# irfanICMLL/structure_knowledge_distillation

Measured on AMD Instinct MI355X. Metric: distillation-step images/sec @512x512 (Pi+Pa+Ho), higher is better.
Workload: dtype f32; 1 GPU; BASELINE configs[2]: ResNet18-PSPNet student + frozen ResNet101-PSPNet teacher, Pi+Pa+Ho (SAGAN D, spectral norm, WGAN-GP), batch 8 per GPU, 512x512, 19 classes; global_batch=8, parallelism=dp1

## Files before the change

### include/skd_eval.h

```cpp
#ifndef SKD_EVAL_H_
#define SKD_EVAL_H_

#include "skd.h"

#ifdef __cplusplus
extern "C" {
#endif

int skd_seg_sliding(int T, int C, int h, int w, int tile_h, int tile_w, int H, int W, const float *logits,
                    const int *tiles, const int64_t *target, int ignore_index, const uint8_t *remap, uint8_t *pred,
                    double *probs, int64_t *confusion, skd_stream_t stream);

#ifdef __cplusplus
}
#endif

#endif
```

### structure_knowledge_distillation_amd/_lib.py

```python
import ctypes
import os
import re

_HERE = os.path.dirname(os.path.abspath(__file__))
LIB_PATH = os.path.join(_HERE, "libskd_hip.so")
HEADER_PATH = os.path.normpath(os.path.join(_HERE, "..", "include", "skd.h"))
EXT_HEADER_PATH = os.path.normpath(os.path.join(_HERE, "..", "include", "skd_eval.h"))

_c = ctypes
_P = _c.c_void_p
_I = _c.c_int
_L = _c.c_int64
_F = _c.c_float
_D = _c.c_double

SIGNATURES = {
    "skd_abi_version": (_I, []),
    "skd_target_arch": (_I, []),
    "skd_bn_mean_var": (_I, [_I, _I, _I, _P, _P, _P, _P]),
    "skd_bn_forward": (_I, [_I, _I, _I, _P, _P, _P, _P, _P, _P, _P, _F, _P]),
    "skd_bn_edz_eydz": (_I, [_I, _I, _I, _P, _P, _P, _P, _P, _P, _F, _P]),
    "skd_bn_backward": (_I, [_I, _I, _I, _P, _P, _P, _P, _P, _P, _P, _P, _P, _P, _F, _P]),
    "skd_leaky_relu": (_I, [_L, _P, _F, _P]),
    "skd_leaky_relu_backward": (_I, [_L, _P, _P, _F, _P]),
    "skd_elu": (_I, [_L, _P, _P]),
    "skd_elu_backward": (_I, [_L, _P, _P, _P]),
    "skd_elu_inv": (_I, [_L, _P, _P]),
    "skd_abn_workspace_floats": (_L, [_I, _I, _I]),
    "skd_abn_forward_train": (_I, [_I, _I, _I, _P, _P, _P, _P, _P, _P, _P, _F, _F, _I, _F, _P, _P]),
    "skd_abn_stats": (_I, [_I, _I, _I, _P, _P, _P, _P, _P]),
    "skd_abn_apply": (_I, [_I, _I, _I, _P, _P, _P, _P, _P, _F, _I, _F, _P]),
    "skd_abn_apply_residual": (_I, [_I, _I, _I, _P, _P, _P, _P, _P, _P, _F, _I, _F, _P]),
    "skd_abn_apply_to": (_I, [_I, _I, _I, _P, _P, _P, _P, _P, _P, _P, _F, _I, _F, _P]),
    "skd_abn_forward_train_to": (_I, [_I, _I, _I, _P, _P, _P, _P, _P, _P, _P, _P, _P, _F, _F, _I, _F, _P, _P]),
    "skd_abn_relu_backward_reduce": (_I, [_I, _I, _I, _P, _P, _P, _P, _P, _P, _P, _F, _P, _P]),
    "skd_abn_relu_backward_dx": (_I, [_I, _I, _I, _P, _P, _P, _P, _P, _P, _P, _P, _P, _P, _P, _P, _F, _P]),
    "skd_abn_apply_nhwc": (_I, [_L, _I, _P, _P, _P, _P, _P, _P, _F, _I, _F, _P]),
    "skd_abn_nhwc_workspace_floats": (_L, [_L, _I]),
    "skd_abn_stats_nhwc": (_I, [_L, _I, _P, _P, _P, _P, _P]),
    "skd_abn_apply_nhwc_to": (_I, [_L, _I, _P, _P, _P, _P, _P, _P, _P, _F, _I, _F, _P]),
    "skd_abn_forward_train_nhwc": (_I, [_L, _I, _P, _P, _P, _P, _P, _P, _P, _P, _P, _F, _F, _I, _F, _P, _P]),
    "skd_abn_backward_reduce_nhwc": (_I, [_L, _I, _P, _P, _P, _P, _P, _P, _F, _I, _F, _P, _P]),
    "skd_abn_backward_dx_nhwc": (_I, [_L, _I, _P, _P, _P, _P, _P, _P, _P, _P, _P, _P, _F, _I, _F, _I, _P]),
    "skd_abn_relu_backward_reduce_nhwc": (_I, [_L, _I, _P, _P, _P, _P, _P, _P, _P, _F, _P, _P]),
    "skd_abn_relu_backward_reduce_nhwc_x": (_I, [_L, _I, _P, _P, _P, _P, _P, _P, _P, _P, _F, _P, _P]),
    "skd_abn_relu_backward_dx_nhwc_x": (_I, [_L, _I, _P, _P, _P, _P, _P, _P, _P, _P, _P, _P, _P, _F, _I, _P]),
    "skd_abn_backward_nhwc": (_I, [_L, _I, _P, _P, _P, _P, _P, _P, _P, _P, _P, _P, _F, _I, _F, _I, _P, _P]),
    "skd_abn_relu_backward_nhwc": (_I, [_L, _I, _P, _P, _P, _P, _P, _P, _P, _P, _P, _P, _P, _P, _P, _F, _I, _P, _P]),
    "skd_abn_relu_backward_dx_nhwc": (_I, [_L, _I, _P, _P, _P, _P, _P, _P, _P, _P, _P, _P, _P, _P, _F, _I, _P]),
    "skd_abn_combine_stats": (_I, [_I, _I, _P, _P, _I, _P, _P, _P, _P, _F, _D, _P]),
    "skd_abn_update_running": (_I, [_I, _P, _P, _P, _P, _F, _D, _P]),
    "skd_abn_backward_reduce": (_I, [_I, _I, _I, _P, _P, _P, _P, _P, _P, _F, _I, _F, _P, _P]),
    "skd_abn_backward_dx": (_I, [_I, _I, _I, _P, _P, _P, _P, _P, _P, _P, _P, _P, _P, _F, _I, _F, _P]),
    "skd_abn_backward": (_I, [_I, _I, _I, _P, _P, _P, _P, _P, _P, _P, _P, _P, _P, _F, _I, _F, _I, _P, _P]),
    "skd_pixelwise_workspace_floats": (_L, [_I, _I]),
    "skd_pixelwise_loss": (_I, [_I, _I, _I, _P, _P, _P, _P, _P, _P]),
    "skd_maxpool_argmax": (_I, [_I, _I, _I, _I, _I, _P, _P, _P, _P]),
    "skd_pairwise_ldm": (_I, [_I]),
    "skd_channel_l2_normalise": (_I, [_I, _I, _I, _P, _P, _I, _P, _I, _P, _P]),
    "skd_pairwise_workspace_floats": (_L, [_I, _I]),
    "skd_pairwise_gram_loss": (_I, [_I, _I, _I, _I, _I, _P, _P, _P, _P, _P, _P]),
    "skd_pairwise_backward_workspace_floats": (_L, [_I, _I, _I]),
    "skd_pairwise_backward": (_I, [_I, _I, _I, _I, _P, _P, _P, _P, _P, _P, _P]),
    "skd_maxunpool_scatter": (_I, [_I, _I, _I, _I, _I, _P, _L, _P, _P, _P]),
    "skd_maxpool_argmax_nhwc": (_I, [_I, _I, _I, _I, _I, _I, _P, _P, _P, _P]),
    "skd_maxunpool_scatter_nhwc": (_I, [_I, _I, _I, _I, _I, _I, _P, _L, _P, _P, _P]),
    "skd_spectral_workspace_floats": (_L, [_I, _I]),
    "skd_spectral_norm_forward": (_I, [_I, _I, _P, _P, _P, _P, _P, _P, _P]),
    "skd_spectral_norm_backward": (_I, [_I, _I, _P, _P, _P, _P, _P, _P, _P, _P]),
    "skd_spectral_norm_forward_multi": (_I, [_I, _P, _P, _P, _P, _P, _P, _P, _P, _P]),
    "skd_spectral_norm_backward_multi": (_I, [_I, _P, _P, _P, _P, _P, _P, _P, _P, _P, _P]),
    "skd_ce_dsn_workspace_floats": (_L, [_I, _I, _I, _I, _I, _I]),
    "skd_ce_dsn_forward": (_I, [_I, _I, _I, _I, _I, _I, _P, _P, _P, _I, _F, _P, _P, _P, _P, _P]),
    "skd_ppm_pooled_floats": (_L, [_I, _I, _P]),
    "skd_ppm_pool": (_I, [_I, _I, _I, _I, _P, _P, _P, _P]),
    "skd_ppm_pool_backward": (_I, [_I, _I, _I, _I, _P, _P, _P, _P]),
    "skd_ppm_concat": (_I, [_I, _I, _I, _I, _I, _I, _P, _P, _P, _P, _P]),
    "skd_ppm_concat_backward": (_I, [_I, _I, _I, _I, _I, _I, _P, _P, _P, _P]),
    "skd_conv1x1_abn_supported": (_I, [_L, _I, _I]),
    "skd_conv1x1_abn_nhwc": (_I, [_L, _I, _I, _P, _P, _P, _P, _P, _P, _P, _P, _F, _I, _F, _P]),
    "skd_abn_pack_eval_params": (_I, [_I, _P, _P, _P, _P, _F, _P, _P]),
    "skd_conv1x1_abn_pro_nhwc": (_I, [_L, _I, _I, _P, _P, _P, _P, _P, _P, _P, _P, _F, _P, _I, _F, _P]),
    "skd_pairwise_small": (_I, [_I, _I, _I, _I, _P, _P, _P, _P, _P, _P]),
    "skd_cs_transform": (_I, [_I, _I, _I, _P, _P, _P, _P, _P, _P, _P, _P, _P, _I, _I, _P, _I, _P, _I, _P, _P]),
    "skd_ppm_nhwc_workspace_floats": (_L, [_I, _I, _I, _I, _I, _I, _P]),
    "skd_ppm_pool_nhwc": (_I, [_I, _I, _I, _I, _I, _P, _P, _P, _P, _P]),
    "skd_ppm_pool_backward_nhwc": (_I, [_I, _I, _I, _I, _I, _P, _P, _P, _P]),
    "skd_ppm_concat_nhwc": (_I, [_I, _I, _I, _I, _I, _I, _P, _P, _P, _P, _P]),
    "skd_ppm_concat_backward_nhwc": (_I, [_I, _I, _I, _I, _I, _I, _P, _P, _P, _P, _P, _P]),
    "skd_ppm_fold_nhwc_workspace_floats": (_L, [_I, _I, _I, _I, _I, _P]),
    "skd_ppm_fold_nhwc": (_I, [_I, _I, _I, _I, _I, _P, _P, _L, _P, _P]),
    "skd_ppm_fold_backward_nhwc": (_I, [_I, _I, _I, _I, _I, _P, _P, _P, _L, _P, _P]),
    "skd_maxpool3x3s2_nhwc": (_I, [_I, _I, _I, _I, _I, _I, _P, _P, _P, _P]),
    "skd_head1x1_supported": (_I, [_I, _I, _I]),
    "skd_head1x1_forward_nhwc": (_I, [_I, _I, _I, _I, _P, _P, _P, _P, _P]),
    "skd_head1x1_backward_workspace_floats": (_L, [_I, _I, _I, _I]),
    "skd_head1x1_backward_nhwc": (_I, [_I, _I, _I, _I, _P, _P, _P, _P, _P, _P, _P, _P]),
    "skd_maxpool3x3s2_backward_nhwc": (_I, [_I, _I, _I, _I, _I, _I, _P, _P, _P, _P]),
    "skd_abn_relu_maxpool3x3s2_nhwc": (_I, [_I, _I, _I, _I, _I, _I, _P, _P, _P, _P, _P, _F, _P, _P, _P]),
    "skd_abn_relu_maxpool3x3s2_backward_reduce_nhwc": (_I, [_I, _I, _I, _I, _I, _I, _P, _P, _P, _P, _P, _P, _P, _P, _P, _F, _P, _P]),
    "skd_abn_relu_maxpool3x3s2_backward_dx_nhwc": (_I, [_I, _I, _I, _I, _I, _I, _P, _P, _P, _P, _P, _P, _P, _P, _P, _P, _P, _P, _F,
                                                         _I, _P]),
    "skd_seg_confusion": (_I, [_I, _I, _I, _I, _I, _I, _P, _P, _I, _P, _P, _P]),
    "skd_sum_f32": (_I, [_L, _P, _P, _F, _P, _P]),
    "skd_sync_handle_bytes": (_I, []),
    "skd_sync_max_floats": (_I, []),
    "skd_sync_create": (_P, [_I, _I, _P]),
    "skd_sync_connect": (_I, [_P, _P]),
    "skd_sync_destroy": (_I, [_P]),
    "skd_sync_all_gather": (_I, [_P, _I, _P, _P, _P]),
    "skd_abn_sync_stats": (_I, [_P, _I, _P, _P, _P, _P, _P, _P, _F, _D, _P]),
    "skd_abn_sync_grad_stats": (_I, [_P, _I, _P, _P, _P]),
    "skd_sync_set_timeout": (_I, [_P, _D]),
    "skd_abn_forward_train_nhwc_sync": (_I, [_P, _L, _I, _P, _P, _P, _P, _P, _P, _P, _P, _P, _P, _F, _F, _I, _F, _D, _P, _P]),
    "skd_abn_backward_nhwc_sync": (_I, [_P, _L, _I, _P, _P, _P, _P, _P, _P, _P, _P, _P, _P, _P, _F, _I, _F, _I, _P, _P]),
    "skd_abn_relu_backward_nhwc_sync": (_I, [_P, _L, _I, _P, _P, _P, _P, _P, _P, _P, _P, _P, _P, _P, _P, _P, _P, _F, _I, _P, _P]),
    "skd_status_words": (_I, []),
    "skd_status_read": (_I, [_P]),
    "skd_status_clear": (_I, []),
    "skd_abn_set_fused_max_workgroups": (_I, [_I]),
    "skd_abn_set_fused": (_I, [_I]),
    "skd_abn_get_fused": (_I, []),
    "skd_abn_set_sync_fused": (_I, [_I]),
    "skd_abn_get_sync_fused": (_I, []),
    "skd_abn_sync_form_counts": (_I, [_P]),
}

EXT_SIGNATURES = {
    "skd_seg_sliding": (_I, [_I, _I, _I, _I, _I, _I, _I, _I, _P, _P, _P, _I, _P, _P, _P, _P, _P]),
}

_lib = None
_test_backend = None


class SkdLibraryError(RuntimeError):
    pass


def header_prototypes(path=HEADER_PATH):
    with open(path) as fh:
        text = re.sub(r"/\*.*?\*/", "", fh.read(), flags=re.S)
    return sorted(set(re.findall(r"\b(skd_[a-z0-9_]+)\s*\(", text)))


def load(path=None):
    global _lib
    if _lib is not None and path is None:
        return _lib
    path = path or LIB_PATH
    if not os.path.exists(path):
        raise SkdLibraryError(
            "libskd_hip.so not found at %s -- build it with "
            "`python -m structure_knowledge_distillation_amd.build` (there is no CPU/eager fallback)" % path)
    try:
        lib = ctypes.CDLL(path)
    except OSError as e:
        raise SkdLibraryError("cannot load %s: %s" % (path, e))
    for table in (SIGNATURES, EXT_SIGNATURES):
        for name, (res, args) in table.items():
            try:
                fn = getattr(lib, name)
            except AttributeError:
                raise SkdLibraryError("libskd_hip.so does not export %s (stale build?)" % name)
            fn.restype = res
            fn.argtypes = args
    if path == LIB_PATH:
        _lib = lib
    return lib


def get():
    if _test_backend is not None:
        return _test_backend
    if _timing is not None:
        return _TimedLib(load())
    return load()


def has_entry(name):
    return hasattr(get(), name)


_timing = None


class _TimedLib:

    def __init__(self, lib):
        self._lib = lib

    def __getattr__(self, name):
        fn = getattr(self._lib, name)
        rec = _timing.get(name) if _timing is not None else None
        if rec is None:
            return fn
        import torch

        def timed(*args):
            e0, e1 = torch.cuda.Event(enable_timing=True), torch.cuda.Event(enable_timing=True)
            e0.record()
            r = fn(*args)
            e1.record()
            rec.append((e0, e1, args[:4]))
            return r
        return timed


def enable_kernel_timing(names):
    global _timing
    _timing = {n: [] for n in names}


def disable_kernel_timing():
    global _timing
    import torch
    out = {}
    if _timing is not None:
        torch.cuda.synchronize()
        for n, recs in _timing.items():
            out[n] = [(e0.elapsed_time(e1), dims) for e0, e1, dims in recs]
    _timing = None
    return out


def install_test_backend(backend):
    global _test_backend
    _test_backend = backend


def test_backend_active():
    return _test_backend is not None


class SkdDeviceError(RuntimeError):
    """A kernel gave up waiting inside a launch (include/skd.h section 13): its outputs are NaN from there on."""


_STATUS_MEANING = {
    0: "a cross-replica InPlace-ABN exchange timed out waiting for a peer rank (SKD_SYNC_TIMEOUT_S): a rank stalled, died or "
       "called the synchronised layers in a different order; statistics are NaN from that exchange on",
    1: "the grid barrier of a one-launch InPlace-ABN pass timed out: its workgroups were not co-resident (device shared with "
       "another grid-barrier launch, partitioned or CU-masked device) -- set SKD_ABN_FUSED=0 or lower "
       "skd_abn_set_fused_max_workgroups",
}


def device_status():
    lib = get()
    n = lib.skd_status_words()
    buf = (ctypes.c_uint * n)()
    if not lib.skd_status_read(ctypes.cast(buf, ctypes.c_void_p)):
        return None
    return list(buf)


def sync_form_counts():
    buf = (ctypes.c_int64 * 2)()
    get().skd_abn_sync_form_counts(ctypes.cast(buf, ctypes.c_void_p))
    return int(buf[0]), int(buf[1])


def raise_on_device_errors():
    words = device_status()
    if words and any(words):
        get().skd_status_clear()
        what = "; ".join("%s (code 0x%08x)" % (_STATUS_MEANING.get(i, "status word %d" % i), w) for i, w in enumerate(words) if w)
        raise SkdDeviceError("structure_knowledge_distillation_amd: " + what)


def check(ok, what):
    if not ok:
        raise RuntimeError("HIP error encountered in %s" % what)


def ptr(t):
    return None if t is None else t.data_ptr()


def int_array(values):
    return (ctypes.c_int * len(values))(*[int(v) for v in values])


def ptr_array(tensors):
    return (ctypes.c_void_p * len(tensors))(*[t.data_ptr() for t in tensors])


def stream_of(t):
    if _test_backend is not None or not t.is_cuda:
        return None
    import torch
    return torch.cuda.current_stream(t.device).cuda_stream


def require_device(*tensors):
    if _test_backend is not None:
        return
    for t in tensors:
        if t is not None and not t.is_cuda:
            raise SkdLibraryError(
                "structure_knowledge_distillation_amd ops run on MI355X only: got a %s tensor "
                "(no CPU fallback exists)" % t.device)
```

### structure_knowledge_distillation_amd/csrc/conv1x1.hip

```cpp
#include <stdio.h>
#include <stdlib.h>

#include <atomic>

#include "skd_common.hpp"

namespace skd {
namespace {

typedef float f32x16 __attribute__((ext_vector_type(16)));
typedef __bf16 bf16x8 __attribute__((ext_vector_type(8)));
typedef __bf16 bf16x2 __attribute__((ext_vector_type(2)));
typedef float f32x2 __attribute__((ext_vector_type(2)));

constexpr int kTM = 128, kTN = 128, kBK = 16, kMinWG = 3;
constexpr int kQK = kBK / 4;
constexpr int kRPP = kThreads / kQK;
constexpr int kRB = kTN / kRPP;
constexpr int kPlaneChunks = 2 * 128;
constexpr int kOperandChunks = 3 * kPlaneChunks;
constexpr int kStageChunks = 2 * kOperandChunks;
constexpr size_t kConvLds = sizeof(uint4) * 2 * kStageChunks;
constexpr int kProMaxK = 512;

__device__ __forceinline__ float inv_std_of(float var, float eps) { return (var != 0.f || eps != 0.f) ? 1.f / sqrtf(var + eps) : 0.f; }

template <int TM>
struct Staging {
  float4 a[TM / kRPP], b[kRB];
};
struct ProParams {
  float4 pm, pi, pg, pb;
};

template <bool PRO, int TM>
__device__ __forceinline__ void stage_load(Staging<TM> &s, const float *__restrict__ X, const float *__restrict__ Wt, int k0,
                                           int gkq, const int64_t (&arow)[TM / kRPP], int64_t wrow0, int K) {
  const float *xa = X + k0 + gkq, *wb = Wt + k0 + gkq;
#pragma unroll
  for (int h = 0; h < TM / kRPP; ++h) s.a[h] = *reinterpret_cast<const float4 *>(xa + arow[h]);
#pragma unroll
  for (int h = 0; h < kRB; ++h) s.b[h] = *reinterpret_cast<const float4 *>(wb + wrow0 + (int64_t)(kRPP * h) * K);
}

__device__ __forceinline__ float pro_one(float x, float m, float is, float g, float b) {
  const float z = __builtin_fmaf((x - m) * is, g, b);
  return z < 0.f ? 0.f : z;
}

__device__ __forceinline__ uint32_t pack_bf16(float x, float y) {
  const f32x2 v = {x, y};
  return __builtin_bit_cast(uint32_t, __builtin_convertvector(v, bf16x2));
}
__device__ __forceinline__ float bf16_lo(uint32_t u) { return __uint_as_float(u << 16); }
__device__ __forceinline__ float bf16_hi(uint32_t u) { return __uint_as_float(u & 0xffff0000u); }

__device__ __forceinline__ void split_store(float4 v, uint2 *dst) {
  uint2 p0, p1, p2;
  p0.x = pack_bf16(v.x, v.y);
  p0.y = pack_bf16(v.z, v.w);
  v.x -= bf16_lo(p0.x); v.y -= bf16_hi(p0.x); v.z -= bf16_lo(p0.y); v.w -= bf16_hi(p0.y);
  p1.x = pack_bf16(v.x, v.y);
  p1.y = pack_bf16(v.z, v.w);
  v.x -= bf16_lo(p1.x); v.y -= bf16_hi(p1.x); v.z -= bf16_lo(p1.y); v.w -= bf16_hi(p1.y);
  p2.x = pack_bf16(v.x, v.y);
  p2.y = pack_bf16(v.z, v.w);
  dst[0] = p0;
  dst[2 * kPlaneChunks] = p1;
  dst[4 * kPlaneChunks] = p2;
}

template <bool PRO, int TM>
__device__ __forceinline__ void stage_store(const Staging<TM> s, uint4 *stage, int srow, const float *ptab, int K, int kq) {
  constexpr int kRA = TM / kRPP;
  uint2 *sa = reinterpret_cast<uint2 *>(stage) + srow, *sb = reinterpret_cast<uint2 *>(stage + kOperandChunks) + srow;
  if (PRO) {
    ProParams pp;
    pp.pm = *reinterpret_cast<const float4 *>(ptab + kq);
    pp.pi = *reinterpret_cast<const float4 *>(ptab + K + kq);
    pp.pg = *reinterpret_cast<const float4 *>(ptab + 2 * K + kq);
    pp.pb = *reinterpret_cast<const float4 *>(ptab + 3 * K + kq);
#pragma unroll
    for (int h = 0; h < kRA; ++h) {
      float4 v = s.a[h];
      v.x = pro_one(v.x, pp.pm.x, pp.pi.x, pp.pg.x, pp.pb.x);
      v.y = pro_one(v.y, pp.pm.y, pp.pi.y, pp.pg.y, pp.pb.y);
      v.z = pro_one(v.z, pp.pm.z, pp.pi.z, pp.pg.z, pp.pb.z);
      v.w = pro_one(v.w, pp.pm.w, pp.pi.w, pp.pg.w, pp.pb.w);
      split_store(v, sa + 2 * kRPP * h);
    }
  } else {
#pragma unroll
    for (int h = 0; h < kRA; ++h) split_store(s.a[h], sa + 2 * kRPP * h);
  }
#pragma unroll
  for (int h = 0; h < kRB; ++h) split_store(s.b[h], sb + 2 * kRPP * h);
}

template <int TM>
__device__ __forceinline__ void tile_mma(const uint4 *stage, f32x16 (&acc)[TM / 64][2]) {
  constexpr int WM = TM / 64;
  const int lane = threadIdx.x & (kWave - 1), wid = threadIdx.x / kWave;
  const int wi = (wid >> 1) * (TM / 2), wj = (wid & 1) * 64;
  const int half = lane >> 5, r = lane & 31;
  const uint4 *pa = stage + half * 128 + ((wi + r) ^ (half * 4));
  const uint4 *pb = stage + kOperandChunks + half * 128 + ((wj + r) ^ (half * 4));
  bf16x8 a[WM][3], b[2][3];
#pragma unroll
  for (int p = 0; p < 3; ++p) {
#pragma unroll
    for (int i = 0; i < WM; ++i) a[i][p] = __builtin_bit_cast(bf16x8, pa[p * kPlaneChunks + 32 * i]);
#pragma unroll
    for (int j = 0; j < 2; ++j) b[j][p] = __builtin_bit_cast(bf16x8, pb[p * kPlaneChunks + 32 * j]);
  }
  constexpr int kPA[6] = {0, 1, 2, 0, 1, 0}, kPB[6] = {2, 1, 0, 1, 0, 0};
#pragma unroll
  for (int t = 0; t < 6; ++t)
#pragma unroll
    for (int i = 0; i < WM; ++i)
#pragma unroll
      for (int j = 0; j < 2; ++j)
        acc[i][j] = __builtin_amdgcn_mfma_f32_32x32x16_bf16(a[i][kPA[t]], b[j][kPB[t]], acc[i][j], 0, 0, 0);
}

template <int ACT, bool HAS_RES, bool FULL, bool NT>
__device__ __forceinline__ void store_block(const f32x16 &acc, const float *__restrict__ R, float *__restrict__ Y, int64_t row0,
                                            int col, int64_t M, int N, float mu, float is, float ga, float be, float slope) {
  const int lane = threadIdx.x & (kWave - 1);
  float rv[16];
  int64_t off[16];
#pragma unroll
  for (int q = 0; q < 16; ++q) {
    const int64_t row = row0 + (q & 3) + 8 * (q >> 2) + 4 * (lane >> 5);
    off[q] = row * N + col;
    rv[q] = 0.f;
    if (HAS_RES && (FULL || row < M)) rv[q] = NT ? __builtin_nontemporal_load(R + off[q]) : R[off[q]];
  }
#pragma unroll
  for (int q = 0; q < 16; ++q) {
    const int64_t row = row0 + (q & 3) + 8 * (q >> 2) + 4 * (lane >> 5);
    float z = ((acc[q] - mu) * is) * ga + be;
    if (HAS_RES) z += rv[q];
    if (ACT == SKD_ACT_RELU) z = z < 0.f ? 0.f : z;
    if (ACT == SKD_ACT_LEAKY_RELU) z = z < 0.f ? z * slope : z;
    if (FULL || row < M) {
      if (NT) __builtin_nontemporal_store(z, Y + off[q]);
      else Y[off[q]] = z;
    }
  }
}

template <int TM, int ACT, bool HAS_RES, bool PRO, bool NT>
__device__ __forceinline__ void conv1x1_tile(const float *__restrict__ X, const float *__restrict__ Wt, const float *__restrict__ R,
                                             float *__restrict__ Y, const float *__restrict__ mean, const float *__restrict__ var,
                                             const float *__restrict__ weight, const float *__restrict__ bias,
                                             const float *__restrict__ ppack, float eps, float slope, int64_t M, int K, int N,
                                             int64_t m0, int n0, uint4 *lds) {
  constexpr int WM = TM / 64, kRA = TM / kRPP;
  f32x16 acc[WM][2];
#pragma unroll
  for (int i = 0; i < WM; ++i)
#pragma unroll
    for (int j = 0; j < 2; ++j)
#pragma unroll
      for (int q = 0; q < 16; ++q) acc[i][j][q] = 0.f;
  const int nk = K / kBK;
  const int gt = threadIdx.x, grow = gt / kQK, gkq = (gt % kQK) * 4;
  const int kh = gkq >> 3;
  const int srow = 2 * (kh * 128 + (grow ^ (kh * 4))) + ((gkq >> 2) & 1);
  int64_t arow[kRA];
#pragma unroll
  for (int h = 0; h < kRA; ++h) {
    const int64_t m = m0 + grow + kRPP * h;
    arow[h] = (m > M - 1 ? M - 1 : m) * K;
  }
  const int64_t wrow0 = (int64_t)(n0 + grow) * K;
  float *ptab = reinterpret_cast<float *>(lds + 2 * kStageChunks);
  if (PRO) {
    for (int i = gt * 4; i < 4 * K; i += kThreads * 4) *reinterpret_cast<float4 *>(ptab + i) = *reinterpret_cast<const float4 *>(ppack + i);
    __syncthreads();
  }
  Staging<TM> st;
  stage_load<PRO, TM>(st, X, Wt, 0, gkq, arow, wrow0, K);
  stage_store<PRO, TM>(st, lds, srow, ptab, K, gkq);
  __syncthreads();
  int stage = 0;
  for (int kt = 0; kt < nk; ++kt) {
    const bool more = kt + 1 < nk;
    if (more) stage_load<PRO, TM>(st, X, Wt, (kt + 1) * kBK, gkq, arow, wrow0, K);
    tile_mma<TM>(lds + stage * kStageChunks, acc);
    if (more) stage_store<PRO, TM>(st, lds + (stage ^ 1) * kStageChunks, srow, ptab, K, (kt + 1) * kBK + gkq);
    __syncthreads();
    stage ^= 1;
  }
  const int lane = threadIdx.x & (kWave - 1), wid = threadIdx.x / kWave;
  const int wi = (wid >> 1) * (TM / 2), wj = (wid & 1) * 64;
  const bool full = m0 + TM <= M;
#pragma unroll
  for (int bj = 0; bj < 2; ++bj) {
    const int col = n0 + wj + bj * 32 + (lane & 31);
    const float mu = mean[col], is = inv_std_of(var[col], eps);
    const float ga = weight != nullptr ? fabsf(weight[col]) + eps : 1.f;
    const float be = bias != nullptr ? bias[col] : 0.f;
#pragma unroll
    for (int bi = 0; bi < WM; ++bi) {
      const int64_t row0 = m0 + wi + bi * 32;
      if (full)
        store_block<ACT, HAS_RES, true, NT>(acc[bi][bj], R, Y, row0, col, M, N, mu, is, ga, be, slope);
      else
        store_block<ACT, HAS_RES, false, NT>(acc[bi][bj], R, Y, row0, col, M, N, mu, is, ga, be, slope);
    }
  }
}

template <int ACT, bool HAS_RES, bool PRO, bool NT>
__global__ __launch_bounds__(kThreads, kMinWG) void conv1x1_abn_kernel(
    const float *__restrict__ X, const float *__restrict__ Wt, const float *__restrict__ R, float *__restrict__ Y,
    const float *__restrict__ mean, const float *__restrict__ var, const float *__restrict__ weight,
    const float *__restrict__ bias, const float *__restrict__ ppack, float eps, float slope, int64_t M, int K, int N,
    int tiles_n, int pm, int ct, int p_full) {
  extern __shared__ __attribute__((aligned(16))) uint4 lds[];
  const int xcd = blockIdx.x & 7, j = blockIdx.x >> 3;
  const int per_group = pm * tiles_n;
  const int group = j / per_group, r = j - group * per_group;
  const int per_chunk = pm * ct;
  const int chunk = r / per_chunk, r2 = r - chunk * per_chunk;
  const int pl = r2 / ct;
  const int tn = chunk * ct + (r2 - pl * ct);
  const int64_t tm = ((int64_t)group * pm + pl) * 8 + xcd;
  if (tn >= tiles_n) return;
  const int n0 = tn * kTN;
  if (tm < p_full) {
    const int64_t m0 = tm * kTM;
    if (m0 >= M) return;
    conv1x1_tile<kTM, ACT, HAS_RES, PRO, NT>(X, Wt, R, Y, mean, var, weight, bias, ppack, eps, slope, M, K, N, m0, n0, lds);
  } else {
    const int64_t m0 = (int64_t)p_full * kTM + (tm - p_full) * (kTM / 2);
    if (m0 >= M) return;
    conv1x1_tile<kTM / 2, ACT, HAS_RES, PRO, NT>(X, Wt, R, Y, mean, var, weight, bias, ppack, eps, slope, M, K, N, m0, n0, lds);
  }
}

__global__ void pack_eval_params_kernel(int K, const float *__restrict__ mean, const float *__restrict__ var,
                                        const float *__restrict__ weight, const float *__restrict__ bias, float eps,
                                        float *__restrict__ pack) {
  const int k = blockIdx.x * blockDim.x + threadIdx.x;
  if (k >= K) return;
  pack[k] = mean[k];
  pack[K + k] = inv_std_of(var[k], eps);
  pack[2 * (int64_t)K + k] = weight != nullptr ? fabsf(weight[k]) + eps : 1.f;
  pack[3 * (int64_t)K + k] = bias != nullptr ? bias[k] : 0.f;
}

static int cu_count(hipStream_t st) {
  static std::atomic<int> cus[64];
  int dev = -1;
  if (hipStreamGetDevice(st, &dev) != hipSuccess) {
    (void)hipGetLastError();
    if (hipGetDevice(&dev) != hipSuccess) return 0;
  }
  if (dev < 0 || dev >= 64) return 0;
  int n = cus[dev].load(std::memory_order_relaxed);
  if (n == 0 && hipDeviceGetAttribute(&n, hipDeviceAttributeMultiprocessorCount, dev) == hipSuccess && n > 0)
    cus[dev].store(n, std::memory_order_relaxed);
  return n > 0 ? n : 0;
}

template <int ACT, bool HAS_RES, bool PRO, bool NT = false>
static int launch(const float *X, const float *Wt, const float *R, float *Y, const float *mean, const float *var,
                  const float *weight, const float *bias, const float *ppack, float eps, float slope, int64_t M, int K, int N,
                  hipStream_t st) {
  static PerDeviceFlag ready;
  bool *rdy = ready.get();
  if (rdy == nullptr) return 0;
  if (!*rdy) {
    if (hipFuncSetAttribute(reinterpret_cast<const void *>(conv1x1_abn_kernel<ACT, HAS_RES, PRO, NT>),
                            hipFuncAttributeMaxDynamicSharedMemorySize, (int)(kConvLds + sizeof(float) * 4 * kProMaxK)) != hipSuccess) return 0;
    *rdy = true;
  }
  const size_t lds_bytes = kConvLds + (PRO ? sizeof(float) * 4 * (size_t)K : 0);
  const int tiles_n = N / kTN;
  const int64_t tiles_m = cdiv(M, kTM);
  const int64_t tile_bytes = (int64_t)kTN * K * sizeof(float);
  int ct = (int)((1 << 20) / tile_bytes), pm = (int)((2 << 20) / tile_bytes);
  if (ct < 1) ct = 1;
  if (pm < 1) pm = 1;
  if (ct >= tiles_n) { ct = tiles_n; pm = 1; }
  else if (!NT) return launch<ACT, HAS_RES, PRO, true>(X, Wt, R, Y, mean, var, weight, bias, ppack, eps, slope, M, K, N, st);
  while (tiles_n % ct) --ct;
  int64_t p_full = tiles_m, panels = tiles_m;
  {
    const int64_t slots = (int64_t)kMinWG * cu_count(st);
    const int64_t tiles = tiles_m * tiles_n;
    if (slots > 0 && tiles > slots && tiles % slots != 0) {
      p_full = (tiles / slots) * slots / tiles_n / 8 * 8;
      const int64_t rest_rows = M - p_full * kTM;
      panels = p_full + cdiv(rest_rows, kTM / 2);
    }
  }
  const int64_t panels_per_xcd = cdiv(cdiv(panels, 8), pm) * pm;
  if (panels_per_xcd * 8 * tiles_n > 2147483647) return 0;
  const int64_t grid = panels_per_xcd * 8 * tiles_n;
  conv1x1_abn_kernel<ACT, HAS_RES, PRO, NT><<<dim3((unsigned)grid), dim3(kThreads), lds_bytes, st>>>(
      X, Wt, R, Y, mean, var, weight, bias, ppack, eps, slope, M, K, N, tiles_n, pm, ct, (int)p_full);
  return ok();
}

}
}

using namespace skd;

extern "C" {

int skd_conv1x1_abn_supported(int64_t M, int K, int N) { return M > 0 && K > 0 && N > 0 && K % kBK == 0 && N % kTN == 0; }

static int conv1x1_dispatch(int64_t M, int K, int N, const float *x, const float *w, const float *residual, float *out,
                            const float *mean, const float *var, const float *weight, const float *bias, const float *ppack,
                            float eps, int activation, float slope, skd_stream_t stream) {
  if (!skd_conv1x1_abn_supported(M, K, N) || !x || !w || !out || !mean || !var) return 0;
  if ((reinterpret_cast<uintptr_t>(x) | reinterpret_cast<uintptr_t>(w) | reinterpret_cast<uintptr_t>(ppack)) & 15) return 0;
  hipStream_t st = as_stream(stream);
#define SKD_C11(A)                                                                                                        \
  if (ppack != nullptr)                                                                                                   \
    return residual ? launch<A, true, true>(x, w, residual, out, mean, var, weight, bias, ppack, eps, slope, M, K, N, st)   \
                    : launch<A, false, true>(x, w, residual, out, mean, var, weight, bias, ppack, eps, slope, M, K, N, st); \
  return residual ? launch<A, true, false>(x, w, residual, out, mean, var, weight, bias, nullptr, eps, slope, M, K, N, st) \
                  : launch<A, false, false>(x, w, residual, out, mean, var, weight, bias, nullptr, eps, slope, M, K, N, st)
  switch (activation) {
    case SKD_ACT_NONE: SKD_C11(SKD_ACT_NONE);
    case SKD_ACT_RELU: SKD_C11(SKD_ACT_RELU);
    case SKD_ACT_LEAKY_RELU: SKD_C11(SKD_ACT_LEAKY_RELU);
    default: return 0;
  }
#undef SKD_C11
}

int skd_conv1x1_abn_nhwc(int64_t M, int K, int N, const float *x, const float *w, const float *residual, float *out,
                         const float *mean, const float *var, const float *weight, const float *bias, float eps,
                         int activation, float slope, skd_stream_t stream) {
  return conv1x1_dispatch(M, K, N, x, w, residual, out, mean, var, weight, bias, nullptr, eps, activation, slope, stream);
}

int skd_abn_pack_eval_params(int K, const float *mean, const float *var, const float *weight, const float *bias, float eps,
                             float *pack, skd_stream_t stream) {
  if (K <= 0 || !mean || !var || !pack) return 0;
  pack_eval_params_kernel<<<dim3((unsigned)cdiv(K, 256)), dim3(256), 0, as_stream(stream)>>>(K, mean, var, weight, bias, eps, pack);
  return ok();
}

int skd_conv1x1_abn_pro_nhwc(int64_t M, int K, int N, const float *x, const float *w, const float *residual, float *out,
                             const float *mean, const float *var, const float *weight, const float *bias, float eps,
                             const float *ppack, int activation, float slope, skd_stream_t stream) {
  if (!ppack || K > kProMaxK) return 0;
  return conv1x1_dispatch(M, K, N, x, w, residual, out, mean, var, weight, bias, ppack, eps, activation, slope, stream);
}

}
```

### structure_knowledge_distillation_amd/functional.py

```python
import ctypes

import torch
from torch.autograd import Function
from torch.autograd.function import once_differentiable

from . import _lib


def _f32c(t, what):
    if t.dtype != torch.float32:
        raise TypeError("%s: fp32 tensors only (got %s)" % (what, t.dtype))
    return t if t.is_contiguous() else t.contiguous()


class _PixelWise(Function):
    @staticmethod
    def forward(ctx, logits_s, logits_t):
        _lib.require_device(logits_s, logits_t)
        assert logits_s.shape == logits_t.shape, "the output dim of teacher and student differ"
        s, t = _f32c(logits_s, "pixel_wise_loss"), _f32c(logits_t, "pixel_wise_loss")
        n, c = s.shape[0], s.shape[1]
        hw = s.numel() // max(1, n * c)
        lib, st = _lib.get(), _lib.stream_of(s)
        loss = s.new_empty(())
        need_grad = ctx.needs_input_grad[0]
        grad = torch.empty_like(s) if need_grad else None
        ws = s.new_empty((max(1, lib.skd_pixelwise_workspace_floats(n, hw)),))
        _lib.check(lib.skd_pixelwise_loss(n, c, hw, s.data_ptr(), t.data_ptr(), loss.data_ptr(),
                                          _lib.ptr(grad), ws.data_ptr(), st), "skd_pixelwise_loss")
        ctx.save_for_backward(grad)
        return loss

    @staticmethod
    @once_differentiable
    def backward(ctx, g):
        (grad,) = ctx.saved_tensors
        return (grad * g if grad is not None else None), None


def pixel_wise_loss(logits_s, logits_t):
    return _PixelWise.apply(logits_s, logits_t.detach())


class _CrossEntropyDSN(Function):
    @staticmethod
    def forward(ctx, logits_main, logits_dsn, target, ignore_index, aux_weight):
        _lib.require_device(logits_main, logits_dsn, target)
        lm = _f32c(logits_main, "cross_entropy_dsn")
        ld = _f32c(logits_dsn, "cross_entropy_dsn") if logits_dsn is not None else None
        if target.dtype != torch.int64:
            raise TypeError("cross_entropy_dsn: int64 target expected (got %s)" % target.dtype)
        tg = target if target.is_contiguous() else target.contiguous()
        b, c, h, w = lm.shape
        if ld is not None and ld.shape != lm.shape:
            raise ValueError("main and dsn logits differ in shape")
        if tg.dim() != 3 or tg.shape[0] != b:
            raise ValueError("target must be (B, H, W)")
        H, W = tg.shape[1], tg.shape[2]
        lib, st = _lib.get(), _lib.stream_of(lm)
        need_m = ctx.needs_input_grad[0]
        need_d = ld is not None and ctx.needs_input_grad[1]
        loss = lm.new_empty(())
        gm = torch.empty_like(lm) if need_m else None
        gd = torch.empty_like(ld) if need_d else None
        ws = lm.new_empty((max(8, lib.skd_ce_dsn_workspace_floats(b, c, h, w, H, W)),))
        _lib.check(lib.skd_ce_dsn_forward(b, c, h, w, H, W, lm.data_ptr(), _lib.ptr(ld), tg.data_ptr(),
                                          int(ignore_index), float(aux_weight), loss.data_ptr(), _lib.ptr(gm),
                                          _lib.ptr(gd), ws.data_ptr(), st), "skd_ce_dsn_forward")
        ctx.save_for_backward(gm, gd)
        return loss

    @staticmethod
    @once_differentiable
    def backward(ctx, g):
        gm, gd = ctx.saved_tensors
        return (gm * g if gm is not None else None), (gd * g if gd is not None else None), None, None, None


def cross_entropy_dsn(logits_main, logits_dsn, target, ignore_index=255, aux_weight=0.4):
    return _CrossEntropyDSN.apply(logits_main, logits_dsn, target, ignore_index, aux_weight)


def _is_cl(t):
    return (t.dim() == 4 and t.shape[1] % 4 == 0 and not t.is_contiguous()
            and t.is_contiguous(memory_format=torch.channels_last))


def _cl(t):
    return t if t.is_contiguous(memory_format=torch.channels_last) else t.contiguous(memory_format=torch.channels_last)


def _new_cl(ref, b, c, h, w):
    return ref.new_empty((b, h, w, c), dtype=torch.float32).permute(0, 3, 1, 2)


class _PPMPool(Function):

    @staticmethod
    def forward(ctx, x, sizes):
        _lib.require_device(x)
        if x.dtype != torch.float32:
            raise TypeError("ppm_pool: fp32 tensors only (got %s)" % x.dtype)
        ctx.cl = _is_cl(x)
        if ctx.cl:
            b, c, h, w = x.shape
            lib, st = _lib.get(), _lib.stream_of(x)
            arr = _lib.int_array(sizes)
            total = lib.skd_ppm_pooled_floats(b * c, len(sizes), arr)
            if total <= 0:
                raise ValueError("ppm_pool: bad pyramid sizes %r" % (sizes,))
            buf = x.new_empty((total,))
            ws = x.new_empty((max(1, lib.skd_ppm_nhwc_workspace_floats(b, c, 0, h, w, len(sizes), arr)),))
            _lib.check(lib.skd_ppm_pool_nhwc(b, c, h, w, len(sizes), arr, x.data_ptr(), buf.data_ptr(), ws.data_ptr(), st),
                       "skd_ppm_pool_nhwc")
            ctx.geom = (b, c, h, w, tuple(sizes))
            outs, off = [], 0
            for s_ in sizes:
                n = b * c * s_ * s_
                outs.append(buf[off:off + n].view(b, s_, s_, c).permute(0, 3, 1, 2))
                off += n
            return tuple(outs)
        x = _f32c(x, "ppm_pool")
        b, c, h, w = x.shape
        lib, st = _lib.get(), _lib.stream_of(x)
        arr = _lib.int_array(sizes)
        total = lib.skd_ppm_pooled_floats(b * c, len(sizes), arr)
        if total <= 0:
            raise ValueError("ppm_pool: bad pyramid sizes %r" % (sizes,))
        buf = x.new_empty((total,))
        _lib.check(lib.skd_ppm_pool(b * c, h, w, len(sizes), arr, x.data_ptr(), buf.data_ptr(), st), "skd_ppm_pool")
        ctx.geom = (b, c, h, w, tuple(sizes))
        outs, off = [], 0
        for s_ in sizes:
            n = b * c * s_ * s_
            outs.append(buf[off:off + n].view(b, c, s_, s_))
            off += n
        return tuple(outs)

    @staticmethod
    @once_differentiable
    def backward(ctx, *grads):
        b, c, h, w, sizes = ctx.geom
        ref = next(g for g in grads if g is not None)
        if ctx.cl:
            flat = torch.cat([(_cl(g).permute(0, 2, 3, 1) if g is not None else ref.new_zeros((b, s_, s_, c))).reshape(-1)
                              for g, s_ in zip(grads, sizes)]).to(torch.float32)
            dx = _new_cl(ref, b, c, h, w)
            lib, st = _lib.get(), _lib.stream_of(flat)
            _lib.check(lib.skd_ppm_pool_backward_nhwc(b, c, h, w, len(sizes), _lib.int_array(sizes), flat.data_ptr(),
                                                      dx.data_ptr(), st), "skd_ppm_pool_backward_nhwc")
            return dx, None
        flat = torch.cat([(g if g is not None else ref.new_zeros((b, c, s_, s_))).reshape(-1)
                          for g, s_ in zip(grads, sizes)]).to(torch.float32)
        dx = ref.new_empty((b, c, h, w), dtype=torch.float32)
        lib, st = _lib.get(), _lib.stream_of(flat)
        _lib.check(lib.skd_ppm_pool_backward(b * c, h, w, len(sizes), _lib.int_array(sizes), flat.data_ptr(),
                                             dx.data_ptr(), st), "skd_ppm_pool_backward")
        return dx, None


def ppm_pool(x, sizes=(1, 2, 3, 6)):
    return _PPMPool.apply(x, tuple(int(s_) for s_ in sizes))


class _PPMConcat(Function):

    @staticmethod
    def forward(ctx, feats, *priors):
        _lib.require_device(feats, *priors)
        ctx.cl = _is_cl(feats) and feats.dtype == torch.float32 and all(p.dtype == torch.float32 and p.shape[1] % 4 == 0 for p in priors)
        if ctx.cl:
            b, cf, h, w = feats.shape
            cout = priors[0].shape[1]
            sizes = []
            for p in priors:
                if p.shape[0] != b or p.shape[1] != cout or p.shape[2] != p.shape[3]:
                    raise ValueError("ppm_concat: priors must be (B, Cout, s, s)")
                sizes.append(p.shape[2])
            priors = [_cl(p) for p in priors]
            lib, st = _lib.get(), _lib.stream_of(feats)
            cat = _new_cl(feats, b, len(priors) * cout + cf, h, w)
            _lib.check(lib.skd_ppm_concat_nhwc(b, cout, cf, h, w, len(sizes), _lib.int_array(sizes), _lib.ptr_array(priors),
                                               feats.data_ptr(), cat.data_ptr(), st), "skd_ppm_concat_nhwc")
            ctx.geom = (b, cout, cf, h, w, tuple(sizes))
            return cat
        feats = _f32c(feats, "ppm_concat")
        priors = [_f32c(p, "ppm_concat") for p in priors]
        b, cf, h, w = feats.shape
        cout = priors[0].shape[1]
        sizes = []
        for p in priors:
            if p.shape[0] != b or p.shape[1] != cout or p.shape[2] != p.shape[3]:
                raise ValueError("ppm_concat: priors must be (B, Cout, s, s)")
            sizes.append(p.shape[2])
        lib, st = _lib.get(), _lib.stream_of(feats)
        cat = feats.new_empty((b, len(priors) * cout + cf, h, w))
        _lib.check(lib.skd_ppm_concat(b, cout, cf, h, w, len(sizes), _lib.int_array(sizes), _lib.ptr_array(priors),
                                      feats.data_ptr(), cat.data_ptr(), st), "skd_ppm_concat")
        ctx.geom = (b, cout, cf, h, w, tuple(sizes))
        return cat

    @staticmethod
    @once_differentiable
    def backward(ctx, gcat):
        b, cout, cf, h, w, sizes = ctx.geom
        if ctx.cl:
            gcat = _cl(gcat.to(torch.float32))
            lib, st = _lib.get(), _lib.stream_of(gcat)
            arr = _lib.int_array(sizes)
            need_p = any(ctx.needs_input_grad[1:])
            gfeats = _new_cl(gcat, b, cf, h, w) if ctx.needs_input_grad[0] else None
            gpriors = [_new_cl(gcat, b, cout, s_, s_) for s_ in sizes] if need_p else None
            ws = gcat.new_empty((max(1, lib.skd_ppm_nhwc_workspace_floats(b, 0, cout, h, w, len(sizes), arr)),)) if need_p else None
            _lib.check(lib.skd_ppm_concat_backward_nhwc(b, cout, cf, h, w, len(sizes), arr, gcat.data_ptr(),
                                                        _lib.ptr_array(gpriors) if need_p else None, _lib.ptr(gfeats),
                                                        _lib.ptr(ws), st), "skd_ppm_concat_backward_nhwc")
            return (gfeats,) + (tuple(gpriors) if need_p else (None,) * len(sizes))
        gcat = _f32c(gcat, "ppm_concat backward")
        lib, st = _lib.get(), _lib.stream_of(gcat)
        gfeats = gcat[:, len(sizes) * cout:] if ctx.needs_input_grad[0] else None
        gpriors = [None] * len(sizes)
        if any(ctx.needs_input_grad[1:]):
            gpriors = [gcat.new_empty((b, cout, s_, s_)) for s_ in sizes]
            _lib.check(lib.skd_ppm_concat_backward(b, cout, cf, h, w, len(sizes), _lib.int_array(sizes),
                                                   gcat.data_ptr(), _lib.ptr_array(gpriors), st),
                       "skd_ppm_concat_backward")
        return (gfeats,) + tuple(gpriors)


def ppm_concat(priors, feats):
    return _PPMConcat.apply(feats, *priors)


def _fold_block_ptrs(z_all, b, cout, sizes):
    ptrs, row = [], 0
    ld = z_all.shape[1]
    for k, s_ in enumerate(sizes):
        ptrs.append(z_all.data_ptr() + 4 * (row * ld + k * 9 * cout))
        row += b * s_ * s_
    return (ctypes.c_void_p * len(ptrs))(*ptrs), ld


class _PPMFold(Function):

    @staticmethod
    def forward(ctx, base, sizes, z_all):
        _lib.require_device(base, z_all)
        b, cout, h, w = base.shape
        if cout % 4 or not base.is_contiguous(memory_format=torch.channels_last) or base.dtype != torch.float32:
            raise ValueError("ppm_fold: base must be a float32 channels-last (B, Cout, H, W) tensor")
        rows = b * sum(s_ * s_ for s_ in sizes)
        if z_all.dtype != torch.float32 or not z_all.is_contiguous() or tuple(z_all.shape) != (rows, len(sizes) * 9 * cout):
            raise ValueError("ppm_fold: Z must be a contiguous float32 (B * sum s^2, L * 9 * Cout) tensor")
        lib, st = _lib.get(), _lib.stream_of(base)
        ptrs, ld = _fold_block_ptrs(z_all, b, cout, sizes)
        _lib.check(lib.skd_ppm_fold_nhwc(b, cout, h, w, len(sizes), _lib.int_array(sizes), ptrs, ld, base.data_ptr(), st),
                   "skd_ppm_fold_nhwc")
        ctx.geom = (b, cout, h, w, tuple(sizes))
        ctx.zshape = z_all.shape
        ctx.mark_dirty(base)
        return base

    @staticmethod
    @once_differentiable
    def backward(ctx, gout):
        b, cout, h, w, sizes = ctx.geom
        gout = _cl(gout.to(torch.float32))
        gz = None
        if ctx.needs_input_grad[2]:
            lib, st = _lib.get(), _lib.stream_of(gout)
            arr = _lib.int_array(sizes)
            gz = gout.new_zeros(ctx.zshape)
            ptrs, ld = _fold_block_ptrs(gz, b, cout, sizes)
            ws = gout.new_empty((max(1, lib.skd_ppm_fold_nhwc_workspace_floats(b, cout, h, w, len(sizes), arr)),))
            _lib.check(lib.skd_ppm_fold_backward_nhwc(b, cout, h, w, len(sizes), arr, gout.data_ptr(), ptrs, ld,
                                                      ws.data_ptr(), st), "skd_ppm_fold_backward_nhwc")
        return gout if ctx.needs_input_grad[0] else None, None, gz


def ppm_fold_supported(feats, sizes):
    return (feats.is_cuda or _lib.test_backend_active()) and feats.dtype == torch.float32 and feats.dim() == 4 \
        and _is_cl(feats) and 3 * sum(sizes) <= 64 and len(sizes) <= 4


def ppm_fold_bottleneck(priors, feats, weight, cache=None):
    import torch.nn.functional as F
    cm = priors[0].shape[1]
    n_prior = len(priors) * cm
    cout = weight.shape[0]
    sizes = tuple(int(p.shape[2]) for p in priors)
    key = (weight.data_ptr(), weight._version, tuple(weight.shape))
    mats = cache.get("mats") if cache is not None and cache.get("key") == key else None
    if mats is None:
        wf = weight[:, n_prior:].contiguous(memory_format=torch.channels_last)
        w_all = weight[:, :n_prior].reshape(cout, len(priors), cm, 3, 3).permute(2, 1, 3, 4, 0).reshape(cm, len(priors) * 9 * cout)
        mats = (wf, w_all)
        if cache is not None and not (torch.is_grad_enabled() and weight.requires_grad):
            cache["key"], cache["mats"] = key, mats
    wf, w_all = mats
    base = F.conv2d(feats, wf, None, 1, 1)
    p_all = torch.cat([_cl(p).permute(0, 2, 3, 1).reshape(-1, cm) for p in priors], 0)
    return _PPMFold.apply(base, sizes, torch.mm(p_all, w_all))


class _MaxPool3x3s2(Function):

    @staticmethod
    def forward(ctx, x, oh, ow):
        _lib.require_device(x)
        b, c, h, w = x.shape
        lib, st = _lib.get(), _lib.stream_of(x)
        y = _new_cl(x, b, c, oh, ow)
        need = ctx.needs_input_grad[0]
        arg = torch.empty((b, oh, ow, c), dtype=torch.uint8, device=x.device) if need else None
        _lib.check(lib.skd_maxpool3x3s2_nhwc(b, c, h, w, oh, ow, x.data_ptr(), y.data_ptr(), _lib.ptr(arg), st), "skd_maxpool3x3s2_nhwc")
        ctx.geom = (b, c, h, w, oh, ow)
        if need:
            ctx.save_for_backward(arg)
        return y

    @staticmethod
    @once_differentiable
    def backward(ctx, gy):
        b, c, h, w, oh, ow = ctx.geom
        (arg,) = ctx.saved_tensors
        gy = _cl(gy.to(torch.float32))
        lib, st = _lib.get(), _lib.stream_of(gy)
        dx = _new_cl(gy, b, c, h, w)
        _lib.check(lib.skd_maxpool3x3s2_backward_nhwc(b, c, h, w, oh, ow, gy.data_ptr(), arg.data_ptr(), dx.data_ptr(), st),
                   "skd_maxpool3x3s2_backward_nhwc")
        return dx, None, None


def _pool_out(n, ceil_mode):
    o = (n + 2 - 3 + (1 if ceil_mode else 0)) // 2 + 1
    if ceil_mode and (o - 1) * 2 >= n + 1:
        o -= 1
    return o


stem_pool_out = _pool_out


def is_stem_pool(pool):
    def _pair(v):
        return tuple(v) if isinstance(v, (tuple, list)) else (v, v)
    return (isinstance(pool, torch.nn.MaxPool2d) and _pair(pool.kernel_size) == (3, 3) and _pair(pool.stride) == (2, 2)
            and _pair(pool.padding) == (1, 1) and _pair(pool.dilation) == (1, 1) and not pool.return_indices)


def max_pool_stem(x, pool):
    if (x.dtype == torch.float32 and _is_cl(x) and (x.is_cuda or _lib.test_backend_active()) and is_stem_pool(pool)):
        return _MaxPool3x3s2.apply(x, _pool_out(x.shape[2], pool.ceil_mode), _pool_out(x.shape[3], pool.ceil_mode))
    return pool(x)


class _Head1x1(Function):

    @staticmethod
    def forward(ctx, x, weight, bias):
        _lib.require_device(x, weight, bias)
        b, k, h, w = x.shape
        c = weight.shape[0]
        lib, st = _lib.get(), _lib.stream_of(x)
        wt = weight.reshape(c, k)
        wt = wt if wt.is_contiguous() else wt.contiguous()
        out = x.new_empty((b, c, h, w))
        _lib.check(lib.skd_head1x1_forward_nhwc(b, h * w, k, c, x.data_ptr(), wt.data_ptr(), _lib.ptr(bias), out.data_ptr(), st),
                   "skd_head1x1_forward_nhwc")
        ctx.save_for_backward(x, weight)
        ctx.has_bias = bias is not None
        return out

    @staticmethod
    @once_differentiable
    def backward(ctx, g):
        x, weight = ctx.saved_tensors
        b, k, h, w = x.shape
        c = weight.shape[0]
        need_x, need_w, need_b = ctx.needs_input_grad[0], ctx.needs_input_grad[1], ctx.has_bias and ctx.needs_input_grad[2]
        g = g if (g.dtype == torch.float32 and g.is_contiguous()) else g.to(torch.float32).contiguous()
        lib, st = _lib.get(), _lib.stream_of(x)
        wt = weight.reshape(c, k)
        wt = wt if wt.is_contiguous() else wt.contiguous()
        gx = _new_cl(x, b, k, h, w) if need_x else None
        gw = torch.empty_like(wt) if need_w else None
        gb = x.new_empty((c,)) if need_b else None
        ws = x.new_empty((max(1, lib.skd_head1x1_backward_workspace_floats(b, h * w, k, c)),))
        _lib.check(lib.skd_head1x1_backward_nhwc(b, h * w, k, c, x.data_ptr(), wt.data_ptr(), g.data_ptr(), _lib.ptr(gx), _lib.ptr(gw),
                                                 _lib.ptr(gb), ws.data_ptr(), st), "skd_head1x1_backward_nhwc")
        return gx, (gw.view_as(weight) if gw is not None else None), gb


def head1x1_supported(x, conv):
    if not (x.dtype == torch.float32 and x.dim() == 4 and _is_cl(x) and (x.is_cuda or _lib.test_backend_active())):
        return False
    if not (conv.kernel_size == (1, 1) and conv.stride == (1, 1) and conv.padding == (0, 0) and conv.dilation == (1, 1)
            and conv.groups == 1 and conv.padding_mode == "zeros" and conv.weight.dtype == torch.float32):
        return False
    grad = torch.is_grad_enabled() and (x.requires_grad or conv.weight.requires_grad
                                        or (conv.bias is not None and conv.bias.requires_grad))
    return bool(_lib.get().skd_head1x1_supported(conv.in_channels, conv.out_channels, 1 if grad else 0))


def head1x1(x, conv):
    return _Head1x1.apply(x, conv.weight, conv.bias)


def blas_1x1_bn_supported(x, conv):
    return (not torch.is_grad_enabled() and x.dtype == torch.float32 and x.dim() == 4
            and x.is_contiguous(memory_format=torch.channels_last) and conv.kernel_size == (1, 1) and conv.stride == (1, 1)
            and conv.padding == (0, 0) and conv.groups == 1 and conv.bias is None
            and conv.in_channels >= 128 and conv.out_channels >= 128)


def conv1x1_bn_blas(x, conv, bn, relu):
    key = tuple((t.data_ptr(), t._version) for t in (conv.weight, bn.weight, bn.bias, bn.running_mean, bn.running_var) if t is not None)
    fold = getattr(bn, "_blas_fold", None)
    if fold is None or fold[0] != key:
        gamma = (bn.weight.abs() + bn.eps) if bn.weight is not None else torch.ones_like(bn.running_var)
        scale = gamma / torch.sqrt(bn.running_var + bn.eps)
        w2 = (conv.weight.reshape(conv.out_channels, conv.in_channels) * scale.view(-1, 1)).contiguous()
        b2 = (bn.bias if bn.bias is not None else torch.zeros_like(scale)) - bn.running_mean * scale
        fold = (key, w2, b2.contiguous())
        bn._blas_fold = fold
    _, w2, b2 = fold
    b, _, h, w = x.shape
    x2 = x.permute(0, 2, 3, 1).reshape(b * h * w, conv.in_channels)
    out = torch._addmm_activation(b2, x2, w2.t()) if relu else torch.addmm(b2, x2, w2.t())
    return out.view(b, h, w, conv.out_channels).permute(0, 3, 1, 2)


def conv1x1_abn_supported(x, conv):
    if not ((x.is_cuda or _lib.test_backend_active()) and x.dtype == torch.float32 and x.dim() == 4
            and x.is_contiguous(memory_format=torch.channels_last)):
        return False
    if not (conv.kernel_size == (1, 1) and conv.stride == (1, 1) and conv.padding == (0, 0) and conv.groups == 1
            and conv.bias is None and conv.weight.dtype == torch.float32):
        return False
    m = x.shape[0] * x.shape[2] * x.shape[3]
    return bool(_lib.get().skd_conv1x1_abn_supported(m, conv.in_channels, conv.out_channels))


def abn_pack_eval_params(bn):
    key = tuple((t.data_ptr(), t._version) if t is not None else None
                for t in (bn.running_mean, bn.running_var, bn.weight, bn.bias)) + (float(bn.eps),)
    cached = getattr(bn, "_skd_eval_pack", None)
    if cached is not None and cached[0] == key:
        return cached[1]
    c = bn.running_mean.numel()
    pack = bn.running_mean.new_empty((4, c))
    _lib.check(_lib.get().skd_abn_pack_eval_params(c, bn.running_mean.data_ptr(), bn.running_var.data_ptr(), _lib.ptr(bn.weight),
                                                   _lib.ptr(bn.bias), float(bn.eps), pack.data_ptr(), _lib.stream_of(pack)),
               "skd_abn_pack_eval_params")
    bn._skd_eval_pack = (key, pack)
    return pack


def conv1x1_abn_eval(x, conv_weight, running_mean, running_var, weight, bias, eps=1e-5, activation="relu", slope=0.01,
                     residual=None, pro=None):
    if torch.is_grad_enabled() and (x.requires_grad or conv_weight.requires_grad):
        raise RuntimeError("conv1x1_abn_eval is inference-only")
    _lib.require_device(x, conv_weight, running_mean, running_var, weight, bias, residual)
    act = {"none": 0, "leaky_relu": 1, "relu": 3}[activation]
    b, k, h, w = x.shape
    n = conv_weight.shape[0]
    out = _new_cl(x, b, n, h, w)
    if residual is not None:
        residual = _cl(residual)
        if tuple(residual.shape) != (b, n, h, w):
            raise ValueError("residual shape %s != output shape %s" % (tuple(residual.shape), (b, n, h, w)))
    wt = conv_weight.reshape(n, k)
    if not wt.is_contiguous():
        wt = wt.contiguous()
    if pro is not None:
        _lib.require_device(pro)
        if pro.dtype != torch.float32 or tuple(pro.shape) != (4, k) or not pro.is_contiguous():
            raise ValueError("pro must be the (4, Cin) fp32 pack of abn_pack_eval_params")
        _lib.check(_lib.get().skd_conv1x1_abn_pro_nhwc(b * h * w, k, n, x.data_ptr(), wt.data_ptr(), _lib.ptr(residual), out.data_ptr(),
                                                       running_mean.data_ptr(), running_var.data_ptr(), _lib.ptr(weight),
                                                       _lib.ptr(bias), float(eps), pro.data_ptr(), act, float(slope),
                                                       _lib.stream_of(x)), "skd_conv1x1_abn_pro_nhwc")
        return out
    _lib.check(_lib.get().skd_conv1x1_abn_nhwc(b * h * w, k, n, x.data_ptr(), wt.data_ptr(), _lib.ptr(residual), out.data_ptr(),
                                               running_mean.data_ptr(), running_var.data_ptr(), _lib.ptr(weight), _lib.ptr(bias),
                                               float(eps), act, float(slope), _lib.stream_of(x)), "skd_conv1x1_abn_nhwc")
    return out


def seg_confusion(logits, target=None, ignore_index=255, confusion=None, want_pred=True):
    _lib.require_device(logits, target, confusion)
    lg = _f32c(logits.detach(), "seg_confusion")
    b, c, h, w = lg.shape
    if target is not None:
        if target.dtype != torch.int64:
            raise TypeError("seg_confusion: int64 target expected (got %s)" % target.dtype)
        tg = target if target.is_contiguous() else target.contiguous()
        H, W = tg.shape[1], tg.shape[2]
        if confusion is None:
            confusion = torch.zeros((c, c), dtype=torch.int64, device=lg.device)
    else:
        tg = None
        H, W = want_pred
    pred = torch.empty((b, H, W), dtype=torch.uint8, device=lg.device) if want_pred else None
    _lib.check(_lib.get().skd_seg_confusion(b, c, h, w, H, W, lg.data_ptr(), _lib.ptr(tg), int(ignore_index), _lib.ptr(pred),
                                            _lib.ptr(confusion), _lib.stream_of(lg)), "skd_seg_confusion")
    return pred, confusion


SEG_SLIDING_MAX_CLASSES = 32


def seg_sliding(logits, tiles, tile_size, out_size, target=None, ignore_index=255, confusion=None, remap=None, want_pred=True,
                want_probs=False):
    _lib.require_device(logits, target, confusion, remap)
    if not _lib.has_entry("skd_seg_sliding"):
        raise NotImplementedError("the active back-end does not provide skd_seg_sliding (include/skd_eval.h)")
    lg = _f32c(logits.detach(), "seg_sliding")
    if lg.dim() != 4:
        raise ValueError("seg_sliding: logits (T, C, h, w) expected (got %s)" % (tuple(lg.shape),))
    nt, c, h, w = lg.shape
    if not 1 <= c <= SEG_SLIDING_MAX_CLASSES:
        raise ValueError("seg_sliding: 1 <= classes <= %d (got %d)" % (SEG_SLIDING_MAX_CLASSES, c))
    (th, tw), (H, W) = (int(v) for v in tile_size), (int(v) for v in out_size)
    if min(th, tw, H, W) <= 0:
        raise ValueError("seg_sliding: tile_size and out_size must be positive")
    if torch.is_tensor(tiles):
        if tiles.dtype != torch.int32 or tiles.device != lg.device or tuple(tiles.shape) != (nt, 4):
            raise TypeError("seg_sliding: tiles tensor must be (%d, 4) int32 on %s" % (nt, lg.device))
        tl = tiles if tiles.is_contiguous() else tiles.contiguous()
    else:
        rows = [tuple(int(v) for v in t) for t in tiles]
        if len(rows) != nt:
            raise ValueError("seg_sliding: %d tiles for %d logit maps" % (len(rows), nt))
        for y1, x1, y2, x2 in rows:
            if not (0 <= y1 < y2 <= H and 0 <= x1 < x2 <= W and y2 - y1 <= th and x2 - x1 <= tw):
                raise ValueError("seg_sliding: tile (%d, %d, %d, %d) does not fit a %d x %d image with %d x %d tiles"
                                 % (y1, x1, y2, x2, H, W, th, tw))
        tl = torch.tensor(rows, dtype=torch.int32).reshape(nt, 4).to(lg.device)
    if target is not None:
        if target.dtype != torch.int64:
            raise TypeError("seg_sliding: int64 target expected (got %s)" % target.dtype)
        if tuple(target.shape[-2:]) != (H, W) or target.numel() != H * W:
            raise ValueError("seg_sliding: target %s does not match out_size %s" % (tuple(target.shape), (H, W)))
        tg = target if target.is_contiguous() else target.contiguous()
        if confusion is None:
            confusion = torch.zeros((c, c), dtype=torch.int64, device=lg.device)
    else:
        tg = None
    if confusion is not None and (confusion.dtype != torch.int64 or tuple(confusion.shape) != (c, c) or not confusion.is_contiguous()):
        raise TypeError("seg_sliding: confusion must be a contiguous (%d, %d) int64 tensor" % (c, c))
    if remap is not None and (remap.dtype != torch.uint8 or remap.numel() != 256 or not remap.is_contiguous()):
        raise TypeError("seg_sliding: remap must be 256 contiguous uint8 entries")
    pred = torch.empty((H, W), dtype=torch.uint8, device=lg.device) if want_pred else None
    probs = torch.empty((H, W, c), dtype=torch.float64, device=lg.device) if want_probs else None
    _lib.check(_lib.get().skd_seg_sliding(nt, c, h, w, th, tw, H, W, lg.data_ptr(), tl.data_ptr(), _lib.ptr(tg), int(ignore_index),
                                          _lib.ptr(remap), _lib.ptr(pred), _lib.ptr(probs), _lib.ptr(confusion), _lib.stream_of(lg)),
               "skd_seg_sliding")
    return pred, probs, confusion


def pool_out_size(n, k):
    return -(-n // k)


class _MaxPoolArgmax(Function):
    @staticmethod
    def forward(ctx, x, kh, kw):
        _lib.require_device(x)
        x = _f32c(x, "max_pool_argmax")
        b, c, h, w = x.shape
        oh, ow = pool_out_size(h, kh), pool_out_size(w, kw)
        lib, st = _lib.get(), _lib.stream_of(x)
        pooled = x.new_empty((b, c, oh, ow))
        need = ctx.needs_input_grad[0]
        index = torch.empty((b, c, oh, ow), dtype=torch.int32, device=x.device) if need else None
        _lib.check(lib.skd_maxpool_argmax(b * c, h, w, kh, kw, x.data_ptr(), pooled.data_ptr(),
                                          _lib.ptr(index), st), "skd_maxpool_argmax")
        ctx.geom = (b, c, h, w, kh, kw)
        ctx.save_for_backward(index)
        return pooled

    @staticmethod
    @once_differentiable
    def backward(ctx, g):
        (index,) = ctx.saved_tensors
        if index is None:
            return None, None, None
        b, c, h, w, kh, kw = ctx.geom
        g = _f32c(g, "max_pool_argmax backward")
        m = g.shape[2] * g.shape[3]
        dx = g.new_empty((b, c, h, w))
        lib, st = _lib.get(), _lib.stream_of(g)
        _lib.check(lib.skd_maxunpool_scatter(b * c, h, w, kh, kw, g.data_ptr(), m, index.data_ptr(),
                                             dx.data_ptr(), st), "skd_maxunpool_scatter")
        return dx, None, None


def max_pool_argmax(x, kh, kw, return_indices=False):
    return _MaxPoolArgmax.apply(x, int(kh), int(kw))


def max_pool_indices(x, kh, kw):
    _lib.require_device(x)
    x = _f32c(x, "max_pool_indices")
    b, c, h, w = x.shape
    oh, ow = pool_out_size(h, kh), pool_out_size(w, kw)
    pooled = x.new_empty((b, c, oh, ow))
    index = torch.empty((b, c, oh, ow), dtype=torch.int32, device=x.device)
    _lib.check(_lib.get().skd_maxpool_argmax(b * c, h, w, int(kh), int(kw), x.data_ptr(), pooled.data_ptr(),
                                             index.data_ptr(), _lib.stream_of(x)), "skd_maxpool_argmax")
    return pooled, index


class _SimDis(Function):

    @staticmethod
    def forward(ctx, f_s, f_t):
        _lib.require_device(f_s, f_t)
        f_s, f_t = _f32c(f_s, "sim_dis"), _f32c(f_t, "sim_dis")
        b, cs = f_s.shape[0], f_s.shape[1]
        ct = f_t.shape[1]
        m = f_t.shape[-1] * f_t.shape[-2]
        assert f_s.shape[0] == f_t.shape[0] and f_s.shape[2:] == f_t.shape[2:]
        lib, st = _lib.get(), _lib.stream_of(f_s)
        ldm = lib.skd_pairwise_ldm(m)
        need = ctx.needs_input_grad[0]
        fh_s = f_s.new_empty((b, cs, ldm))
        fh_t = f_s.new_empty((b, ct, ldm))
        norm_s = f_s.new_empty((b, m)) if need else None
        _lib.check(lib.skd_channel_l2_normalise(b, cs, m, f_s.data_ptr(), fh_s.data_ptr(), ldm,
                                                None, 0, _lib.ptr(norm_s), st),
                   "skd_channel_l2_normalise")
        _lib.check(lib.skd_channel_l2_normalise(b, ct, m, f_t.data_ptr(), fh_t.data_ptr(), ldm,
                                                None, 0, None, st), "skd_channel_l2_normalise")
        g = f_s.new_empty((b, ldm, ldm)) if need else None
        loss = f_s.new_empty(())
        ws = f_s.new_empty((max(1, lib.skd_pairwise_workspace_floats(b, m)),))
        _lib.check(lib.skd_pairwise_gram_loss(b, cs, ct, m, ldm, fh_s.data_ptr(), fh_t.data_ptr(),
                                              _lib.ptr(g), loss.data_ptr(), ws.data_ptr(), st),
                   "skd_pairwise_gram_loss")
        ctx.geom = (tuple(f_s.shape), m, ldm)
        ctx.save_for_backward(fh_s if need else None, g, norm_s)
        return loss

    @staticmethod
    @once_differentiable
    def backward(ctx, gl):
        fh_s, g, norm_s = ctx.saved_tensors
        if g is None:
            return None, None
        shape, m, ldm = ctx.geom
        b, cs = shape[0], shape[1]
        lib, st = _lib.get(), _lib.stream_of(g)
        gl = gl.to(torch.float32).contiguous()
        dp = g.new_empty((b, cs, ldm))
        ws = g.new_empty((max(1, lib.skd_pairwise_backward_workspace_floats(b, cs, m)),))
        _lib.check(lib.skd_pairwise_backward(b, cs, m, ldm, fh_s.data_ptr(), g.data_ptr(),
                                             norm_s.data_ptr(), gl.data_ptr(), dp.data_ptr(), ws.data_ptr(), st),
                   "skd_pairwise_backward")
        return dp[:, :, :m].reshape(shape), None


def sim_dis(f_s, f_t):
    return _SimDis.apply(f_s, f_t.detach())


def _channels_last_quads(t):
    return (t.dim() == 4 and t.shape[1] % 4 == 0 and t.is_contiguous(memory_format=torch.channels_last) and not t.is_contiguous()
            and t.data_ptr() % 16 == 0)


def _pool_feature(lib, t, kh, kw, pooled, index, st):
    b, c, h, w = t.shape
    if _channels_last_quads(t):
        _lib.check(lib.skd_maxpool_argmax_nhwc(b, c, h, w, kh, kw, t.data_ptr(), pooled.data_ptr(), _lib.ptr(index), st),
                   "skd_maxpool_argmax_nhwc")
        return t
    t = t if t.is_contiguous() else t.contiguous()
    _lib.check(lib.skd_maxpool_argmax(b * c, h, w, kh, kw, t.data_ptr(), pooled.data_ptr(), _lib.ptr(index), st), "skd_maxpool_argmax")
    return t


def _unpool_feature(lib, nhwc, geom, dp, ldp, index, st):
    b, cs, h, w, kh, kw = geom
    if nhwc:
        dx = torch.empty_strided((b, cs, h, w), (h * w * cs, 1, w * cs, cs), dtype=dp.dtype, device=dp.device)
        _lib.check(lib.skd_maxunpool_scatter_nhwc(b, cs, h, w, kh, kw, dp.data_ptr(), ldp, index.data_ptr(), dx.data_ptr(), st),
                   "skd_maxunpool_scatter_nhwc")
        return dx
    dx = dp.new_empty((b, cs, h, w))
    _lib.check(lib.skd_maxunpool_scatter(b * cs, h, w, kh, kw, dp.data_ptr(), ldp, index.data_ptr(), dx.data_ptr(), st),
               "skd_maxunpool_scatter")
    return dx


class _PairWise(Function):

    @staticmethod
    def forward(ctx, feat_s, feat_t, kh, kw):
        _lib.require_device(feat_s, feat_t)
        for t in (feat_s, feat_t):
            if t.dtype != torch.float32:
                raise TypeError("pair_wise_loss: fp32 tensors only (got %s)" % t.dtype)
        b, cs, h, w = feat_s.shape
        ct = feat_t.shape[1]
        assert feat_t.shape[0] == b and tuple(feat_t.shape[2:]) == (h, w)
        oh, ow = pool_out_size(h, kh), pool_out_size(w, kw)
        m = oh * ow
        lib, st = _lib.get(), _lib.stream_of(feat_s)
        need = ctx.needs_input_grad[0]
        ctx.nhwc = _channels_last_quads(feat_s)
        if m <= 64:
            p_s, p_t = feat_s.new_empty((b, cs, m)), feat_s.new_empty((b, ct, m))
            index = torch.empty((b, cs, m), dtype=torch.int32, device=feat_s.device) if need else None
            _pool_feature(lib, feat_s, kh, kw, p_s, index, st)
            _pool_feature(lib, feat_t, kh, kw, p_t, None, st)
            loss = feat_s.new_empty(())
            dp = feat_s.new_empty((b, cs, m)) if need else None
            ws = feat_s.new_empty((b,))
            _lib.check(lib.skd_pairwise_small(b, cs, ct, m, p_s.data_ptr(), p_t.data_ptr(), loss.data_ptr(), _lib.ptr(dp),
                                              ws.data_ptr(), st), "skd_pairwise_small")
            ctx.geom = (b, cs, h, w, kh, kw, m, 0, 0)
            ctx.small = True
            ctx.save_for_backward(dp, index)
            return loss
        ctx.small = False
        ldm = lib.skd_pairwise_ldm(m)
        p_s = feat_s.new_empty((b, cs, m))
        p_t = feat_s.new_empty((b, ct, m))
        index = torch.empty((b, cs, m), dtype=torch.int32, device=feat_s.device) if need else None
        _pool_feature(lib, feat_s, kh, kw, p_s, index, st)
        _pool_feature(lib, feat_t, kh, kw, p_t, None, st)
        fh_s = feat_s.new_empty((b, cs, ldm))
        fh_t = feat_s.new_empty((b, ct, ldm))
        norm_s = feat_s.new_empty((b, m)) if need else None
        _lib.check(lib.skd_channel_l2_normalise(b, cs, m, p_s.data_ptr(), fh_s.data_ptr(), ldm,
                                                None, 0, _lib.ptr(norm_s), st),
                   "skd_channel_l2_normalise")
        _lib.check(lib.skd_channel_l2_normalise(b, ct, m, p_t.data_ptr(), fh_t.data_ptr(), ldm,
                                                None, 0, None, st), "skd_channel_l2_normalise")
        g = feat_s.new_empty((b, ldm, ldm)) if need else None
        loss = feat_s.new_empty(())
        ws = feat_s.new_empty((max(1, lib.skd_pairwise_workspace_floats(b, m)),))
        _lib.check(lib.skd_pairwise_gram_loss(b, cs, ct, m, ldm, fh_s.data_ptr(), fh_t.data_ptr(),
                                              _lib.ptr(g), loss.data_ptr(), ws.data_ptr(), st),
                   "skd_pairwise_gram_loss")
        ctx.geom = (b, cs, h, w, kh, kw, m, ldm, 0)
        ctx.save_for_backward(fh_s if need else None, g, norm_s, index)
        return loss

    @staticmethod
    @once_differentiable
    def backward(ctx, gl):
        if ctx.small:
            dp, index = ctx.saved_tensors
            if dp is None:
                return None, None, None, None
            b, cs, h, w, kh, kw, m, _, _ = ctx.geom
            lib, st = _lib.get(), _lib.stream_of(dp)
            dpg = dp * gl.to(torch.float32)
            return _unpool_feature(lib, ctx.nhwc, (b, cs, h, w, kh, kw), dpg, m, index, st), None, None, None
        fh_s, g, norm_s, index = ctx.saved_tensors
        if g is None:
            return None, None, None, None
        b, cs, h, w, kh, kw, m, ldm, _ = ctx.geom
        lib, st = _lib.get(), _lib.stream_of(g)
        gl = gl.to(torch.float32).contiguous()
        dp = g.new_empty((b, cs, ldm))
        ws = g.new_empty((max(1, lib.skd_pairwise_backward_workspace_floats(b, cs, m)),))
        _lib.check(lib.skd_pairwise_backward(b, cs, m, ldm, fh_s.data_ptr(), g.data_ptr(),
                                             norm_s.data_ptr(), gl.data_ptr(), dp.data_ptr(), ws.data_ptr(), st),
                   "skd_pairwise_backward")
        return _unpool_feature(lib, ctx.nhwc, (b, cs, h, w, kh, kw), dp, ldm, index, st), None, None, None


def pair_wise_loss(feat_s, feat_t, kh, kw):
    return _PairWise.apply(feat_s, feat_t.detach(), int(kh), int(kw))


class _SpectralNormalize(Function):

    @staticmethod
    def forward(ctx, w_bar, u, v):
        _lib.require_device(w_bar, u, v)
        wb = _f32c(w_bar, "spectral_normalize")
        h = wb.shape[0]
        wd = wb.numel() // h
        if not (u.is_contiguous() and v.is_contiguous()) or u.numel() != h or v.numel() != wd:
            raise ValueError("spectral_normalize: u/v must be contiguous vectors of length (out, in*kh*kw)")
        lib, st = _lib.get(), _lib.stream_of(wb)
        sigma = wb.new_empty(())
        w = torch.empty_like(wb)
        ws = wb.new_empty((max(1, lib.skd_spectral_workspace_floats(h, wd)),))
        _lib.check(lib.skd_spectral_norm_forward(h, wd, wb.data_ptr(), u.data_ptr(), v.data_ptr(),
                                                 sigma.data_ptr(), w.data_ptr(), ws.data_ptr(), st),
                   "skd_spectral_norm_forward")
        ctx.u, ctx.v = u, v
        ctx.save_for_backward(wb, sigma)
        return w

    @staticmethod
    @once_differentiable
    def backward(ctx, gw):
        wb, sigma = ctx.saved_tensors
        h = wb.shape[0]
        wd = wb.numel() // h
        gw = _f32c(gw, "spectral_normalize backward")
        lib, st = _lib.get(), _lib.stream_of(wb)
        gwb = torch.empty_like(wb)
        ws = wb.new_empty((max(1, lib.skd_spectral_workspace_floats(h, wd)),))
        _lib.check(lib.skd_spectral_norm_backward(h, wd, wb.data_ptr(), ctx.u.data_ptr(), ctx.v.data_ptr(),
                                                  sigma.data_ptr(), gw.data_ptr(), gwb.data_ptr(),
                                                  ws.data_ptr(), st), "skd_spectral_norm_backward")
        return gwb, None, None


def spectral_normalize(w_bar, u, v):
    return _SpectralNormalize.apply(w_bar, u, v)


class _SpectralNormalizeMulti(Function):

    @staticmethod
    def forward(ctx, us, vs, *w_bars):
        _lib.require_device(*w_bars, *us, *vs)
        wbs = [_f32c(w, "spectral_normalize_multi") for w in w_bars]
        hs = [w.shape[0] for w in wbs]
        ws_ = [w.numel() // h for w, h in zip(wbs, hs)]
        for u, v, h, wd in zip(us, vs, hs, ws_):
            if not (u.is_contiguous() and v.is_contiguous()) or u.numel() != h or v.numel() != wd:
                raise ValueError("spectral_normalize: u/v must be contiguous vectors of length (out, in*kh*kw)")
        lib, st = _lib.get(), _lib.stream_of(wbs[0])
        sigmas = wbs[0].new_empty((len(wbs),))
        outs = [torch.empty_like(w) for w in wbs]
        work = wbs[0].new_empty((sum(max(1, lib.skd_spectral_workspace_floats(h, wd)) for h, wd in zip(hs, ws_)),))
        sig = [sigmas[k:k + 1] for k in range(len(wbs))]
        _lib.check(lib.skd_spectral_norm_forward_multi(len(wbs), _lib.int_array(hs), _lib.int_array(ws_), _lib.ptr_array(wbs),
                                                       _lib.ptr_array(us), _lib.ptr_array(vs), _lib.ptr_array(sig),
                                                       _lib.ptr_array(outs), work.data_ptr(), st), "skd_spectral_norm_forward_multi")
        ctx.us, ctx.vs, ctx.hs, ctx.ws_ = list(us), list(vs), hs, ws_
        ctx.save_for_backward(sigmas, *wbs)
        return tuple(outs)

    @staticmethod
    @once_differentiable
    def backward(ctx, *gws):
        sigmas, *wbs = ctx.saved_tensors
        lib, st = _lib.get(), _lib.stream_of(wbs[0])
        gws = [torch.zeros_like(w) if g is None else _f32c(g, "spectral_normalize backward") for g, w in zip(gws, wbs)]
        gwbs = [torch.empty_like(w) for w in wbs]
        work = wbs[0].new_empty((sum(max(1, lib.skd_spectral_workspace_floats(h, wd)) for h, wd in zip(ctx.hs, ctx.ws_)),))
        sig = [sigmas[k:k + 1] for k in range(len(wbs))]
        _lib.check(lib.skd_spectral_norm_backward_multi(len(wbs), _lib.int_array(ctx.hs), _lib.int_array(ctx.ws_), _lib.ptr_array(wbs),
                                                        _lib.ptr_array(ctx.us), _lib.ptr_array(ctx.vs), _lib.ptr_array(sig),
                                                        _lib.ptr_array(gws), _lib.ptr_array(gwbs), work.data_ptr(), st),
                   "skd_spectral_norm_backward_multi")
        return (None, None) + tuple(gwbs)


def spectral_normalize_multi(w_bars, us, vs):
    return _SpectralNormalizeMulti.apply(list(us), list(vs), *w_bars)


def spectral_power_iteration(w_bar, u, v):
    _lib.require_device(w_bar, u, v)
    wb = _f32c(w_bar.detach(), "spectral_power_iteration")
    h = wb.shape[0]
    wd = wb.numel() // h
    lib, st = _lib.get(), _lib.stream_of(wb)
    sigma = wb.new_empty(())
    ws = wb.new_empty((max(1, lib.skd_spectral_workspace_floats(h, wd)),))
    _lib.check(lib.skd_spectral_norm_forward(h, wd, wb.data_ptr(), u.data_ptr(), v.data_ptr(),
                                             sigma.data_ptr(), None, ws.data_ptr(), st),
               "skd_spectral_norm_forward")
    return sigma
```

### structure_knowledge_distillation_amd/networks/pspnet_combine.py

```python
import functools

import torch
import torch.nn as nn
import torch.nn.functional as F

from .. import functional as SF
from ..libs import InPlaceABN, InPlaceABNSync

affine_par = True
BatchNorm2d = functools.partial(InPlaceABNSync, activation="none")


def _fused(module, x):
    return x.dtype == torch.float32 and (module.training or not torch.is_grad_enabled())


FUSED_TAIL = True
BLAS_TAILS = True
HEAD_KERNEL = True
STEM_FUSED = True
PSP_FOLD = True


def _fused_tail(x):
    return FUSED_TAIL and not torch.is_grad_enabled() and x.dtype == torch.float32


def _blas_tail(module, x):
    return BLAS_TAILS and not module.training and not torch.is_grad_enabled()


class _ClassifierConvFn(torch.autograd.Function):

    @staticmethod
    def forward(ctx, x, weight, bias, stride, padding, dilation):
        ctx.save_for_backward(x, weight)
        ctx.conv = (stride, padding, dilation)
        return F.conv2d(x, weight, bias, stride, padding, dilation)

    @staticmethod
    def backward(ctx, g):
        x, weight = ctx.saved_tensors
        stride, padding, dilation = ctx.conv
        gx = torch.nn.grad.conv2d_input(x.shape, weight, g, stride, padding, dilation) if ctx.needs_input_grad[0] else None
        gw = torch.nn.grad.conv2d_weight(x, weight.shape, g, stride, padding, dilation) if ctx.needs_input_grad[1] else None
        gb = g.permute(0, 2, 3, 1).sum(2).sum((0, 1)) if ctx.needs_input_grad[2] else None
        return gx, gw, gb, None, None, None


class ClassifierConv(nn.Conv2d):

    def _plain(self):
        return (self.groups == 1 and self.padding_mode == "zeros" and not isinstance(self.padding, str)
                and not self.transposed and tuple(self.output_padding) == (0, 0))

    def forward(self, x):
        if HEAD_KERNEL and SF.head1x1_supported(x, self):
            return SF.head1x1(x, self)
        if (self.bias is None or not self._plain()
                or not (torch.is_grad_enabled() and (x.requires_grad or self.weight.requires_grad))):
            return super().forward(x)
        return _ClassifierConvFn.apply(x, self.weight, self.bias, self.stride, self.padding, self.dilation)


def conv3x3(in_planes, out_planes, stride=1):
    return nn.Conv2d(in_planes, out_planes, kernel_size=3, stride=stride, padding=1, bias=False)


class BasicBlock(nn.Module):
    expansion = 1

    def __init__(self, inplanes, planes, stride=1, dilation=1, downsample=None, multi_grid=1):
        super().__init__()
        d = dilation * multi_grid
        self.conv1 = nn.Conv2d(inplanes, planes, 3, stride, d, d, bias=False)
        self.bn1 = BatchNorm2d(planes)
        self.relu = nn.ReLU(inplace=False)
        self.conv2 = nn.Conv2d(planes, planes, 3, 1, d, d, bias=False)
        self.bn2 = BatchNorm2d(planes)
        self.relu_inplace = nn.ReLU(inplace=True)
        self.downsample = downsample

    def forward(self, x):
        if _fused(self, x):
            out = self.bn1.forward_relu(self.conv1(x))
            residual = self.downsample(x) if self.downsample is not None else x
            return self.bn2.forward_relu(self.conv2(out), residual)
        out = self.relu(self.bn1(self.conv1(x)))
        out = self.bn2(self.conv2(out))
        residual = self.downsample(x) if self.downsample is not None else x
        return self.relu_inplace(out + residual)


class Bottleneck(nn.Module):
    expansion = 4

    def __init__(self, inplanes, planes, stride=1, dilation=1, downsample=None, fist_dilation=1, multi_grid=1):
        super().__init__()
        d = dilation * multi_grid
        self.conv1 = nn.Conv2d(inplanes, planes, 1, bias=False)
        self.bn1 = BatchNorm2d(planes)
        self.conv2 = nn.Conv2d(planes, planes, 3, stride, d, d, bias=False)
        self.bn2 = BatchNorm2d(planes)
        self.conv3 = nn.Conv2d(planes, planes * 4, 1, bias=False)
        self.bn3 = BatchNorm2d(planes * 4)
        self.relu = nn.ReLU(inplace=False)
        self.relu_inplace = nn.ReLU(inplace=True)
        self.downsample = downsample
        self.dilation = dilation
        self.stride = stride

    def forward(self, x):
        if _fused(self, x):
            blas = _blas_tail(self, x)
            if blas and SF.blas_1x1_bn_supported(x, self.conv1):
                out = SF.conv1x1_bn_blas(x, self.conv1, self.bn1, relu=True)
            else:
                out = self.bn1.forward_relu(self.conv1(x))
            c2 = self.conv2(out)
            tail = (not self.training and _fused_tail(x) and SF.conv1x1_abn_supported(c2, self.conv3) and self.conv3.in_channels <= 512
                    and getattr(self.bn2, "activation", None) == "none" and getattr(self.bn3, "activation", None) == "none")
            if not tail:
                out = self.bn2.forward_relu(c2)
            if self.downsample is None:
                residual = x
            elif (blas and len(self.downsample) == 2 and SF.blas_1x1_bn_supported(x, self.downsample[0])
                  and getattr(self.downsample[1], "activation", None) == "none"):
                residual = SF.conv1x1_bn_blas(x, self.downsample[0], self.downsample[1], relu=False)
            else:
                residual = self.downsample(x)
            if tail:
                return SF.conv1x1_abn_eval(c2, self.conv3.weight, self.bn3.running_mean, self.bn3.running_var, self.bn3.weight,
                                           self.bn3.bias, self.bn3.eps, "relu", residual=residual,
                                           pro=SF.abn_pack_eval_params(self.bn2))
            return self.bn3.forward_relu(self.conv3(out), residual)
        out = self.relu(self.bn1(self.conv1(x)))
        out = self.relu(self.bn2(self.conv2(out)))
        out = self.bn3(self.conv3(out))
        residual = self.downsample(x) if self.downsample is not None else x
        return self.relu_inplace(out + residual)


def _conv1x1_as_mm(conv, x):
    if not (conv.kernel_size == (1, 1) and conv.stride == (1, 1) and conv.padding == (0, 0) and conv.groups == 1
            and x.dtype == torch.float32 and x.dim() == 4 and x.is_contiguous(memory_format=torch.channels_last)):
        return conv(x)
    b, c, h, w = x.shape
    x2, wt = x.permute(0, 2, 3, 1).reshape(b * h * w, c), conv.weight.reshape(conv.out_channels, c).t()
    out = torch.mm(x2, wt) if conv.bias is None else torch.addmm(conv.bias, x2, wt)
    return out.view(b, h, w, conv.out_channels).permute(0, 3, 1, 2)


class PSPModule(nn.Module):

    def __init__(self, features, out_features=512, sizes=(1, 2, 3, 6)):
        super().__init__()
        self.stages = nn.ModuleList([self._make_stage(features, out_features, s) for s in sizes])
        self.bottleneck = nn.Sequential(
            nn.Conv2d(features + len(sizes) * out_features, out_features, 3, padding=1, dilation=1, bias=False),
            InPlaceABNSync(out_features),
            nn.Dropout2d(0.1))

    def _make_stage(self, features, out_features, size):
        return nn.Sequential(nn.AdaptiveAvgPool2d(output_size=(size, size)),
                             nn.Conv2d(features, out_features, 1, bias=False),
                             InPlaceABNSync(out_features))

    def forward(self, feats):
        sizes = []
        for stage in self.stages:
            o = stage[0].output_size
            sizes.append(o[0] if isinstance(o, (tuple, list)) else o)
        nhwc = feats.dim() == 4 and not feats.is_contiguous() and feats.is_contiguous(memory_format=torch.channels_last)
        if (feats.dtype == torch.float32 and len(sizes) <= 4 and (nhwc or feats.size(3) <= 256)
                and min(feats.size(2), feats.size(3)) >= max(sizes)):
            pooled = SF.ppm_pool(feats, sizes)
            if nhwc:
                priors = [stage[2](_conv1x1_as_mm(stage[1], p)) for stage, p in zip(self.stages, pooled)]
            else:
                priors = [stage[2](stage[1](p)) for stage, p in zip(self.stages, pooled)]
            conv = self.bottleneck[0]
            if (nhwc and PSP_FOLD and SF.ppm_fold_supported(feats, sizes) and conv.bias is None
                    and conv.kernel_size == (3, 3) and conv.padding == (1, 1) and conv.stride == (1, 1)
                    and conv.dilation == (1, 1) and conv.groups == 1 and conv.out_channels % 4 == 0
                    and all(p.shape[1] == priors[0].shape[1] for p in priors)):
                if not hasattr(self, "_fold_cache"):
                    self._fold_cache = {}
                out = SF.ppm_fold_bottleneck(priors, feats, conv.weight, self._fold_cache)
                return self.bottleneck[2](self.bottleneck[1](out))
            return self.bottleneck(SF.ppm_concat(priors, feats))
        h, w = feats.size(2), feats.size(3)
        priors = [F.interpolate(stage(feats), size=(h, w), mode="bilinear", align_corners=True)
                  for stage in self.stages] + [feats]
        return self.bottleneck(torch.cat(priors, 1))


class ResNet(nn.Module):
    def __init__(self, block, layers, num_classes):
        self.inplanes = 128
        super().__init__()
        self.conv1 = conv3x3(3, 64, stride=2)
        self.bn1 = BatchNorm2d(64)
        self.relu1 = nn.ReLU(inplace=False)
        self.conv2 = conv3x3(64, 64)
        self.bn2 = BatchNorm2d(64)
        self.relu2 = nn.ReLU(inplace=False)
        self.conv3 = conv3x3(64, 128)
        self.bn3 = BatchNorm2d(128)
        self.relu3 = nn.ReLU(inplace=False)
        self.relu = nn.ReLU(inplace=False)
        self.maxpool = nn.MaxPool2d(kernel_size=3, stride=2, padding=1, ceil_mode=True)
        self.layer1 = self._make_layer(block, 64, layers[0])
        self.layer2 = self._make_layer(block, 128, layers[1], stride=2)
        self.layer3 = self._make_layer(block, 256, layers[2], stride=1, dilation=2)
        self.layer4 = self._make_layer(block, 512, layers[3], stride=1, dilation=4, multi_grid=(1, 1, 1))
        layers = list(layers)
        if layers == [3, 4, 23, 3]:
            feat, mid = 2048, 512
        elif layers == [2, 2, 2, 2]:
            feat, mid = 512, 128
        else:
            raise ValueError("layers should be [3, 4, 23, 3] or [2, 2, 2, 2]")
        self.pspmodule = PSPModule(feat, mid)
        self.head = ClassifierConv(mid, num_classes, 1, 1, 0, bias=True)
        self.dsn = nn.Sequential(
            nn.Conv2d(feat // 2, mid, 3, 1, 1),
            InPlaceABNSync(mid),
            nn.Dropout2d(0.1),
            ClassifierConv(mid, num_classes, 1, 1, 0, bias=True))

    def _make_layer(self, block, planes, blocks, stride=1, dilation=1, multi_grid=1):
        downsample = None
        if stride != 1 or self.inplanes != planes * block.expansion:
            downsample = nn.Sequential(
                nn.Conv2d(self.inplanes, planes * block.expansion, 1, stride, bias=False),
                BatchNorm2d(planes * block.expansion, affine=affine_par))
        grid = lambda i: multi_grid[i % len(multi_grid)] if isinstance(multi_grid, tuple) else 1
        mods = [block(self.inplanes, planes, stride, dilation=dilation, downsample=downsample, multi_grid=grid(0))]
        self.inplanes = planes * block.expansion
        for i in range(1, blocks):
            mods.append(block(self.inplanes, planes, dilation=dilation, multi_grid=grid(i)))
        return nn.Sequential(*mods)

    def forward(self, x):
        if _fused(self, x) and not self.training and getattr(self.bn3, "activation", None) == "none":
            x = self.bn1.forward_relu(self.conv1(x))
            x = self.bn2.forward_relu(self.conv2(x))
            x = self.bn3.forward_relu(SF.max_pool_stem(self.conv3(x), self.maxpool))
        else:
            if _fused(self, x):
                x = self.bn1.forward_relu(self.conv1(x))
                x = self.bn2.forward_relu(self.conv2(x))
                x = (self.bn3.forward_relu_maxpool(self.conv3(x), self.maxpool) if STEM_FUSED
                     else SF.max_pool_stem(self.bn3.forward_relu(self.conv3(x)), self.maxpool))
            else:
                x = self.relu1(self.bn1(self.conv1(x)))
                x = self.relu2(self.bn2(self.conv2(x)))
                x = self.relu3(self.bn3(self.conv3(x)))
                x = SF.max_pool_stem(x, self.maxpool)
        x1 = self.layer1(x)
        x2 = self.layer2(x1)
        x3 = self.layer3(x2)
        if getattr(self, "skip_dsn", False) and not torch.is_grad_enabled():
            x_dsn = None
        elif getattr(self, "dsn_last", None) is not None and not torch.is_grad_enabled():
            x4 = self.layer4(x3)
            x_feat_after_psp = self.pspmodule(x4)
            x = self.head(x_feat_after_psp)
            self.dsn_last(x, x_feat_after_psp)
            x_dsn = self.dsn(x3)
            return [x, x_dsn, x_feat_after_psp, x4, x3, x2, x1]
        else:
            x_dsn = self.dsn(x3)
        x4 = self.layer4(x3)
        x_feat_after_psp = self.pspmodule(x4)
        x = self.head(x_feat_after_psp)
        return [x, x_dsn, x_feat_after_psp, x4, x3, x2, x1]


def Res_pspnet(block=Bottleneck, layers=[3, 4, 23, 3], num_classes=21):
    return ResNet(block, layers, num_classes)
```

Before: 133.0 images/sec.

## Add implicit-GEMM 3x3 conv with split-bf16 MFMA for frozen teacher inference

Adds a new HIP implicit-GEMM 3x3 convolution kernel for NHWC inputs. It splits fp32 activations into three bf16 planes and runs six-term MFMA products with a separate low-order accumulator. Weights are pre-packed once and cached per module, and BN, bias and activation are fused into the epilogue. The kernel is used for the frozen teacher's bottleneck conv2, the DSN head and the PSP fold bottleneck when Cin is at least 256. It also routes some 1x1 conv+BN pairs to the existing split conv1x1 kernel instead of BLAS, and moves shared device helpers into a common header. The aim is to replace generic fp32 convolution on the teacher path with tensor-core math while keeping near-fp32 accuracy.

```diff
diff --git a/include/skd_eval.h b/include/skd_eval.h
--- a/include/skd_eval.h
+++ b/include/skd_eval.h
@@ -11,6 +11,14 @@
                     const int *tiles, const int64_t *target, int ignore_index, const uint8_t *remap, uint8_t *pred,
                     double *probs, int64_t *confusion, skd_stream_t stream);
 
+int skd_conv3x3_split_supported(int Cin, int Cout, int stride, int padding, int dilation, int groups);
+int64_t skd_conv3x3_split_pack_bytes(int Cin, int Cout);
+int skd_conv3x3_split_pack_weights(int Cin, int Cout, const float *w, int64_t stride_n, int64_t stride_c, int64_t stride_y,
+                                   int64_t stride_x, void *pack, int64_t pack_bytes, skd_stream_t stream);
+int skd_conv3x3_split_nhwc(int B, int H, int W, int Cin, int Cout, int dilation, const float *x, const void *wpack, float *out,
+                           const float *conv_bias, const float *mean, const float *var, const float *weight, const float *bias,
+                           float eps, int activation, float slope, int geometry, skd_stream_t stream);
+
 #ifdef __cplusplus
 }
 #endif
diff --git a/structure_knowledge_distillation_amd/_lib.py b/structure_knowledge_distillation_amd/_lib.py
--- a/structure_knowledge_distillation_amd/_lib.py
+++ b/structure_knowledge_distillation_amd/_lib.py
@@ -128,6 +128,10 @@
 
 EXT_SIGNATURES = {
     "skd_seg_sliding": (_I, [_I, _I, _I, _I, _I, _I, _I, _I, _P, _P, _P, _I, _P, _P, _P, _P, _P]),
+    "skd_conv3x3_split_supported": (_I, [_I, _I, _I, _I, _I, _I]),
+    "skd_conv3x3_split_pack_bytes": (_L, [_I, _I]),
+    "skd_conv3x3_split_pack_weights": (_I, [_I, _I, _P, _L, _L, _L, _L, _P, _L, _P]),
+    "skd_conv3x3_split_nhwc": (_I, [_I, _I, _I, _I, _I, _I, _P, _P, _P, _P, _P, _P, _P, _P, _F, _I, _F, _I, _P]),
 }
 
 _lib = None
diff --git a/structure_knowledge_distillation_amd/csrc/conv1x1.hip b/structure_knowledge_distillation_amd/csrc/conv1x1.hip
--- a/structure_knowledge_distillation_amd/csrc/conv1x1.hip
+++ b/structure_knowledge_distillation_amd/csrc/conv1x1.hip
@@ -1,29 +1,12 @@
 #include <stdio.h>
 #include <stdlib.h>
 
-#include <atomic>
-
-#include "skd_common.hpp"
+#include "conv_split_dev.hpp"
 
 namespace skd {
 namespace {
 
-typedef float f32x16 __attribute__((ext_vector_type(16)));
-typedef __bf16 bf16x8 __attribute__((ext_vector_type(8)));
-typedef __bf16 bf16x2 __attribute__((ext_vector_type(2)));
-typedef float f32x2 __attribute__((ext_vector_type(2)));
-
-constexpr int kTM = 128, kTN = 128, kBK = 16, kMinWG = 3;
-constexpr int kQK = kBK / 4;
-constexpr int kRPP = kThreads / kQK;
-constexpr int kRB = kTN / kRPP;
-constexpr int kPlaneChunks = 2 * 128;
-constexpr int kOperandChunks = 3 * kPlaneChunks;
-constexpr int kStageChunks = 2 * kOperandChunks;
-constexpr size_t kConvLds = sizeof(uint4) * 2 * kStageChunks;
 constexpr int kProMaxK = 512;
-
-__device__ __forceinline__ float inv_std_of(float var, float eps) { return (var != 0.f || eps != 0.f) ? 1.f / sqrtf(var + eps) : 0.f; }
 
 template <int TM>
 struct Staging {
@@ -46,28 +29,6 @@
 __device__ __forceinline__ float pro_one(float x, float m, float is, float g, float b) {
   const float z = __builtin_fmaf((x - m) * is, g, b);
   return z < 0.f ? 0.f : z;
-}
-
-__device__ __forceinline__ uint32_t pack_bf16(float x, float y) {
-  const f32x2 v = {x, y};
-  return __builtin_bit_cast(uint32_t, __builtin_convertvector(v, bf16x2));
-}
-__device__ __forceinline__ float bf16_lo(uint32_t u) { return __uint_as_float(u << 16); }
-__device__ __forceinline__ float bf16_hi(uint32_t u) { return __uint_as_float(u & 0xffff0000u); }
-
-__device__ __forceinline__ void split_store(float4 v, uint2 *dst) {
-  uint2 p0, p1, p2;
-  p0.x = pack_bf16(v.x, v.y);
-  p0.y = pack_bf16(v.z, v.w);
-  v.x -= bf16_lo(p0.x); v.y -= bf16_hi(p0.x); v.z -= bf16_lo(p0.y); v.w -= bf16_hi(p0.y);
-  p1.x = pack_bf16(v.x, v.y);
-  p1.y = pack_bf16(v.z, v.w);
-  v.x -= bf16_lo(p1.x); v.y -= bf16_hi(p1.x); v.z -= bf16_lo(p1.y); v.w -= bf16_hi(p1.y);
-  p2.x = pack_bf16(v.x, v.y);
-  p2.y = pack_bf16(v.z, v.w);
-  dst[0] = p0;
-  dst[2 * kPlaneChunks] = p1;
-  dst[4 * kPlaneChunks] = p2;
 }
 
 template <bool PRO, int TM>
@@ -97,59 +58,6 @@
   for (int h = 0; h < kRB; ++h) split_store(s.b[h], sb + 2 * kRPP * h);
 }
 
-template <int TM>
-__device__ __forceinline__ void tile_mma(const uint4 *stage, f32x16 (&acc)[TM / 64][2]) {
-  constexpr int WM = TM / 64;
-  const int lane = threadIdx.x & (kWave - 1), wid = threadIdx.x / kWave;
-  const int wi = (wid >> 1) * (TM / 2), wj = (wid & 1) * 64;
-  const int half = lane >> 5, r = lane & 31;
-  const uint4 *pa = stage + half * 128 + ((wi + r) ^ (half * 4));
-  const uint4 *pb = stage + kOperandChunks + half * 128 + ((wj + r) ^ (half * 4));
-  bf16x8 a[WM][3], b[2][3];
-#pragma unroll
-  for (int p = 0; p < 3; ++p) {
-#pragma unroll
-    for (int i = 0; i < WM; ++i) a[i][p] = __builtin_bit_cast(bf16x8, pa[p * kPlaneChunks + 32 * i]);
-#pragma unroll
-    for (int j = 0; j < 2; ++j) b[j][p] = __builtin_bit_cast(bf16x8, pb[p * kPlaneChunks + 32 * j]);
-  }
-  constexpr int kPA[6] = {0, 1, 2, 0, 1, 0}, kPB[6] = {2, 1, 0, 1, 0, 0};
-#pragma unroll
-  for (int t = 0; t < 6; ++t)
-#pragma unroll
-    for (int i = 0; i < WM; ++i)
-#pragma unroll
-      for (int j = 0; j < 2; ++j)
-        acc[i][j] = __builtin_amdgcn_mfma_f32_32x32x16_bf16(a[i][kPA[t]], b[j][kPB[t]], acc[i][j], 0, 0, 0);
-}
-
-template <int ACT, bool HAS_RES, bool FULL, bool NT>
-__device__ __forceinline__ void store_block(const f32x16 &acc, const float *__restrict__ R, float *__restrict__ Y, int64_t row0,
-                                            int col, int64_t M, int N, float mu, float is, float ga, float be, float slope) {
-  const int lane = threadIdx.x & (kWave - 1);
-  float rv[16];
-  int64_t off[16];
-#pragma unroll
-  for (int q = 0; q < 16; ++q) {
-    const int64_t row = row0 + (q & 3) + 8 * (q >> 2) + 4 * (lane >> 5);
-    off[q] = row * N + col;
-    rv[q] = 0.f;
-    if (HAS_RES && (FULL || row < M)) rv[q] = NT ? __builtin_nontemporal_load(R + off[q]) : R[off[q]];
-  }
-#pragma unroll
-  for (int q = 0; q < 16; ++q) {
-    const int64_t row = row0 + (q & 3) + 8 * (q >> 2) + 4 * (lane >> 5);
-    float z = ((acc[q] - mu) * is) * ga + be;
-    if (HAS_RES) z += rv[q];
-    if (ACT == SKD_ACT_RELU) z = z < 0.f ? 0.f : z;
-    if (ACT == SKD_ACT_LEAKY_RELU) z = z < 0.f ? z * slope : z;
-    if (FULL || row < M) {
-      if (NT) __builtin_nontemporal_store(z, Y + off[q]);
-      else Y[off[q]] = z;
-    }
-  }
-}
-
 template <int TM, int ACT, bool HAS_RES, bool PRO, bool NT>
 __device__ __forceinline__ void conv1x1_tile(const float *__restrict__ X, const float *__restrict__ Wt, const float *__restrict__ R,
                                              float *__restrict__ Y, const float *__restrict__ mean, const float *__restrict__ var,
@@ -166,8 +74,7 @@
       for (int q = 0; q < 16; ++q) acc[i][j][q] = 0.f;
   const int nk = K / kBK;
   const int gt = threadIdx.x, grow = gt / kQK, gkq = (gt % kQK) * 4;
-  const int kh = gkq >> 3;
-  const int srow = 2 * (kh * 128 + (grow ^ (kh * 4))) + ((gkq >> 2) & 1);
+  const int srow = plane_slot(grow, gkq);
   int64_t arow[kRA];
 #pragma unroll
   for (int h = 0; h < kRA; ++h) {
@@ -252,20 +159,6 @@
   pack[3 * (int64_t)K + k] = bias != nullptr ? bias[k] : 0.f;
 }
 
-static int cu_count(hipStream_t st) {
-  static std::atomic<int> cus[64];
-  int dev = -1;
-  if (hipStreamGetDevice(st, &dev) != hipSuccess) {
-    (void)hipGetLastError();
-    if (hipGetDevice(&dev) != hipSuccess) return 0;
-  }
-  if (dev < 0 || dev >= 64) return 0;
-  int n = cus[dev].load(std::memory_order_relaxed);
-  if (n == 0 && hipDeviceGetAttribute(&n, hipDeviceAttributeMultiprocessorCount, dev) == hipSuccess && n > 0)
-    cus[dev].store(n, std::memory_order_relaxed);
-  return n > 0 ? n : 0;
-}
-
 template <int ACT, bool HAS_RES, bool PRO, bool NT = false>
 static int launch(const float *X, const float *Wt, const float *R, float *Y, const float *mean, const float *var,
                   const float *weight, const float *bias, const float *ppack, float eps, float slope, int64_t M, int K, int N,
diff --git a/structure_knowledge_distillation_amd/csrc/conv3x3.hip b/structure_knowledge_distillation_amd/csrc/conv3x3.hip
--- /dev/null
+++ b/structure_knowledge_distillation_amd/csrc/conv3x3.hip
@@ -0,0 +1,260 @@
+#include "conv_split_dev.hpp"
+
+namespace skd {
+namespace {
+
+constexpr int kTileChunks = kOperandChunks;
+constexpr int kBChunksPerThread = kTileChunks / kThreads;
+
+template <int TM>
+struct Staging3 {
+  float4 a[TM / kRPP];
+  uint4 b[kBChunksPerThread];
+};
+
+struct TapCursor {
+  int tap, c0;
+  int64_t shift;
+};
+
+__device__ __forceinline__ int64_t tap_shift(int tap, int W, int dil, int Cin) {
+  const int ty = tap / 3, tx = tap - 3 * ty;
+  return ((int64_t)(ty - 1) * W + (tx - 1)) * dil * Cin;
+}
+
+template <int TM>
+__device__ __forceinline__ void stage_load3(Staging3<TM> &s, const float *__restrict__ X, const uint4 *__restrict__ bsrc,
+                                            const TapCursor &cur, const int64_t (&abase)[TM / kRPP], const unsigned (&mask)[TM / kRPP]) {
+#pragma unroll
+  for (int h = 0; h < TM / kRPP; ++h) {
+    s.a[h] = make_float4(0.f, 0.f, 0.f, 0.f);
+    if ((mask[h] >> cur.tap) & 1u) s.a[h] = *reinterpret_cast<const float4 *>(X + abase[h] + cur.shift + cur.c0);
+  }
+#pragma unroll
+  for (int p = 0; p < kBChunksPerThread; ++p) s.b[p] = bsrc[p * kPlaneChunks];
+}
+
+template <int TM>
+__device__ __forceinline__ void stage_store3(const Staging3<TM> s, uint4 *stage, int srow) {
+  uint2 *sa = reinterpret_cast<uint2 *>(stage) + srow;
+#pragma unroll
+  for (int h = 0; h < TM / kRPP; ++h) split_store(s.a[h], sa + 2 * kRPP * h);
+  uint4 *sb = stage + kOperandChunks + threadIdx.x;
+#pragma unroll
+  for (int p = 0; p < kBChunksPerThread; ++p) sb[p * kPlaneChunks] = s.b[p];
+}
+
+template <int TM, int ACT>
+__device__ __forceinline__ void conv3x3_tile(const float *__restrict__ X, const uint4 *__restrict__ Bp, float *__restrict__ Y,
+                                             const float *__restrict__ cbias, const float *__restrict__ mean,
+                                             const float *__restrict__ var, const float *__restrict__ weight,
+                                             const float *__restrict__ bias, float eps, float slope, int64_t M, int H, int W,
+                                             int Cin, int N, int dil, int64_t m0, int tn, uint4 *lds) {
+  constexpr int WM = TM / 64, kRA = TM / kRPP;
+  f32x16 acc[WM][2], low[WM][2];
+#pragma unroll
+  for (int i = 0; i < WM; ++i)
+#pragma unroll
+    for (int j = 0; j < 2; ++j)
+#pragma unroll
+      for (int q = 0; q < 16; ++q) acc[i][j][q] = low[i][j][q] = 0.f;
+  const int nk = 9 * (Cin / kBK);
+  const int gt = threadIdx.x, grow = gt / kQK, gkq = (gt % kQK) * 4;
+  const int srow = plane_slot(grow, gkq);
+  int64_t abase[kRA];
+  unsigned mask[kRA];
+  const int64_t hw = (int64_t)H * W;
+#pragma unroll
+  for (int h = 0; h < kRA; ++h) {
+    const int64_t m = m0 + grow + kRPP * h;
+    const bool live = m < M;
+    const int64_t mm = live ? m : 0;
+    const int pix = (int)(mm % hw);
+    const int py = pix / W, px = pix - py * W;
+    unsigned bits = 0;
+#pragma unroll
+    for (int tap = 0; tap < 9; ++tap) {
+      const int64_t y = py + (int64_t)(tap / 3 - 1) * dil, x = px + (int64_t)(tap % 3 - 1) * dil;
+      if (live && y >= 0 && y < H && x >= 0 && x < W) bits |= 1u << tap;
+    }
+    mask[h] = bits;
+    abase[h] = mm * Cin + gkq;
+  }
+  const uint4 *bsrc = Bp + (int64_t)tn * nk * kTileChunks + gt;
+  TapCursor cur = {0, 0, tap_shift(0, W, dil, Cin)};
+  Staging3<TM> st;
+  stage_load3<TM>(st, X, bsrc, cur, abase, mask);
+  stage_store3<TM>(st, lds, srow);
+  __syncthreads();
+  int stage = 0;
+  for (int kt = 0; kt < nk; ++kt) {
+    const bool more = kt + 1 < nk;
+    if (more) {
+      cur.c0 += kBK;
+      if (cur.c0 == Cin) {
+        cur.c0 = 0;
+        ++cur.tap;
+        cur.shift = tap_shift(cur.tap, W, dil, Cin);
+      }
+      stage_load3<TM>(st, X, bsrc + (int64_t)(kt + 1) * kTileChunks, cur, abase, mask);
+    }
+    tile_mma<TM>(lds + stage * kStageChunks, low, acc);
+    if (more) stage_store3<TM>(st, lds + (stage ^ 1) * kStageChunks, srow);
+    __syncthreads();
+    stage ^= 1;
+  }
+  const int lane = threadIdx.x & (kWave - 1), wid = threadIdx.x / kWave;
+  const int wi = (wid >> 1) * (TM / 2), wj = (wid & 1) * 64;
+  const bool full = m0 + TM <= M;
+#pragma unroll
+  for (int bj = 0; bj < 2; ++bj) {
+    const int col = tn * kTN + wj + bj * 32 + (lane & 31);
+    const bool bn = mean != nullptr;
+    const float mu = bn ? mean[col] : 0.f, is = bn ? inv_std_of(var[col], eps) : 1.f;
+    const float ga = bn && weight != nullptr ? fabsf(weight[col]) + eps : 1.f;
+    const float be = bn && bias != nullptr ? bias[col] : 0.f;
+    const float cb = cbias != nullptr ? cbias[col] : 0.f;
+#pragma unroll
+    for (int bi = 0; bi < WM; ++bi) {
+#pragma unroll
+      for (int q = 0; q < 16; ++q) acc[bi][bj][q] += low[bi][bj][q];
+      if (cbias != nullptr) {
+#pragma unroll
+        for (int q = 0; q < 16; ++q) acc[bi][bj][q] += cb;
+      }
+      const int64_t row0 = m0 + wi + bi * 32;
+      if (full)
+        store_block<ACT, false, true, false>(acc[bi][bj], nullptr, Y, row0, col, M, N, mu, is, ga, be, slope);
+      else
+        store_block<ACT, false, false, false>(acc[bi][bj], nullptr, Y, row0, col, M, N, mu, is, ga, be, slope);
+    }
+  }
+}
+
+template <int ACT, bool TALL>
+__global__ __launch_bounds__(kThreads, TALL ? 2 : kMinWG) __attribute__((amdgpu_waves_per_eu(TALL ? 2 : kMinWG, TALL ? 2 : kMinWG)))
+void conv3x3_split_kernel(
+    const float *__restrict__ X, const uint4 *__restrict__ Bp, float *__restrict__ Y, const float *__restrict__ cbias,
+    const float *__restrict__ mean, const float *__restrict__ var, const float *__restrict__ weight,
+    const float *__restrict__ bias, float eps, float slope, int64_t M, int H, int W, int Cin, int N, int dil, int tiles_n,
+    int p_full) {
+  extern __shared__ __attribute__((aligned(16))) uint4 lds[];
+  const int xcd = blockIdx.x & 7, j = blockIdx.x >> 3;
+  const int pl = j / tiles_n, tn = j - pl * tiles_n;
+  const int64_t tm = (int64_t)pl * 8 + xcd;
+  if (TALL && tm < p_full) {
+    const int64_t m0 = tm * kTM;
+    if (m0 >= M) return;
+    conv3x3_tile<kTM, ACT>(X, Bp, Y, cbias, mean, var, weight, bias, eps, slope, M, H, W, Cin, N, dil, m0, tn, lds);
+  } else {
+    const int64_t m0 = (int64_t)p_full * kTM + (tm - p_full) * (kTM / 2);
+    if (m0 >= M) return;
+    conv3x3_tile<kTM / 2, ACT>(X, Bp, Y, cbias, mean, var, weight, bias, eps, slope, M, H, W, Cin, N, dil, m0, tn, lds);
+  }
+}
+
+__global__ void conv3x3_pack_kernel(const float *__restrict__ Wt, int64_t sn, int64_t sc, int64_t sy, int64_t sx, int Cin, int nk,
+                                    int64_t chunks, uint4 *__restrict__ pack) {
+  const int64_t idx = (int64_t)blockIdx.x * blockDim.x + threadIdx.x;
+  if (idx >= chunks) return;
+  const int chunk = (int)(idx % kPlaneChunks);
+  const int64_t tile = idx / kPlaneChunks;
+  const int kt = (int)(tile % nk), tn = (int)(tile / nk);
+  const int kh = chunk >> 7, row = (chunk & 127) ^ (kh * 4);
+  const int k0 = kt * kBK + kh * 8, tap = k0 / Cin, c0 = k0 - tap * Cin;
+  const int ty = tap / 3, tx = tap - 3 * ty;
+  const float *src = Wt + (int64_t)(tn * kTN + row) * sn + ty * sy + tx * sx;
+  float v[8];
+#pragma unroll
+  for (int i = 0; i < 8; ++i) v[i] = src[(c0 + i) * sc];
+  uint2 lo[3], hi[3];
+  split4(make_float4(v[0], v[1], v[2], v[3]), lo[0], lo[1], lo[2]);
+  split4(make_float4(v[4], v[5], v[6], v[7]), hi[0], hi[1], hi[2]);
+#pragma unroll
+  for (int p = 0; p < 3; ++p) pack[(tile * 3 + p) * kPlaneChunks + chunk] = make_uint4(lo[p].x, lo[p].y, hi[p].x, hi[p].y);
+}
+
+template <int ACT, bool TALL>
+static int launch3(const float *X, const uint4 *Bp, float *Y, const float *cbias, const float *mean, const float *var,
+                   const float *weight, const float *bias, float eps, float slope, int64_t M, int H, int W, int Cin, int N, int dil,
+                   int geometry, hipStream_t st) {
+  static PerDeviceFlag ready;
+  bool *rdy = ready.get();
+  if (rdy == nullptr) return 0;
+  if (!*rdy) {
+    if (hipFuncSetAttribute(reinterpret_cast<const void *>(conv3x3_split_kernel<ACT, TALL>),
+                            hipFuncAttributeMaxDynamicSharedMemorySize, (int)kConvLds) != hipSuccess) return 0;
+    *rdy = true;
+  }
+  const int tiles_n = N / kTN;
+  const int64_t tiles_m = cdiv(M, kTM);
+  int64_t p_full = TALL ? tiles_m : 0;
+  if (TALL && geometry == 3) {
+    const int64_t slots = 2 * (int64_t)cu_count(st), tiles = tiles_m * tiles_n;
+    if (slots > 0 && tiles % slots != 0) p_full = (tiles / slots) * slots / tiles_n / 8 * 8;
+  }
+  const int64_t panels = p_full < tiles_m ? p_full + cdiv(M - p_full * kTM, kTM / 2) : tiles_m;
+  const int64_t grid = cdiv(panels, 8) * 8 * tiles_n;
+  if (grid > 2147483647) return 0;
+  conv3x3_split_kernel<ACT, TALL><<<dim3((unsigned)grid), dim3(kThreads), kConvLds, st>>>(
+      X, Bp, Y, cbias, mean, var, weight, bias, eps, slope, M, H, W, Cin, N, dil, tiles_n, (int)p_full);
+  return ok();
+}
+
+template <int ACT>
+static int launch3g(const float *X, const uint4 *Bp, float *Y, const float *cbias, const float *mean, const float *var,
+                    const float *weight, const float *bias, float eps, float slope, int64_t M, int H, int W, int Cin, int N, int dil,
+                    int geometry, hipStream_t st) {
+  if (geometry == 0) geometry = cdiv(M, kTM) * (N / kTN) > 2 * (int64_t)cu_count(st) ? 3 : 2;
+  if (geometry == 1 || geometry == 3)
+    return launch3<ACT, true>(X, Bp, Y, cbias, mean, var, weight, bias, eps, slope, M, H, W, Cin, N, dil, geometry, st);
+  return launch3<ACT, false>(X, Bp, Y, cbias, mean, var, weight, bias, eps, slope, M, H, W, Cin, N, dil, geometry, st);
+}
+
+}
+}
+
+using namespace skd;
+
+extern "C" {
+
+int skd_conv3x3_split_supported(int Cin, int Cout, int stride, int padding, int dilation, int groups) {
+  return Cin > 0 && Cout > 0 && Cin % kBK == 0 && Cout % kTN == 0 && stride == 1 && dilation >= 1 && padding == dilation && groups == 1;
+}
+
+int64_t skd_conv3x3_split_pack_bytes(int Cin, int Cout) {
+  if (!skd_conv3x3_split_supported(Cin, Cout, 1, 1, 1, 1)) return 0;
+  return (int64_t)(Cout / kTN) * (9 * (Cin / kBK)) * kTileChunks * (int64_t)sizeof(uint4);
+}
+
+int skd_conv3x3_split_pack_weights(int Cin, int Cout, const float *w, int64_t stride_n, int64_t stride_c, int64_t stride_y,
+                                   int64_t stride_x, void *pack, int64_t pack_bytes, skd_stream_t stream) {
+  const int64_t need = skd_conv3x3_split_pack_bytes(Cin, Cout);
+  if (need == 0 || !w || !pack || pack_bytes < need || (reinterpret_cast<uintptr_t>(pack) & 15)) return 0;
+  if (stride_n < 0 || stride_c < 0 || stride_y < 0 || stride_x < 0) return 0;
+  const int nk = 9 * (Cin / kBK);
+  const int64_t chunks = (int64_t)(Cout / kTN) * nk * kPlaneChunks;
+  conv3x3_pack_kernel<<<dim3((unsigned)cdiv(chunks, 256)), dim3(256), 0, as_stream(stream)>>>(
+      w, stride_n, stride_c, stride_y, stride_x, Cin, nk, chunks, static_cast<uint4 *>(pack));
+  return ok();
+}
+
+int skd_conv3x3_split_nhwc(int B, int H, int W, int Cin, int Cout, int dilation, const float *x, const void *wpack, float *out,
+                           const float *conv_bias, const float *mean, const float *var, const float *weight, const float *bias,
+                           float eps, int activation, float slope, int geometry, skd_stream_t stream) {
+  if (!skd_conv3x3_split_supported(Cin, Cout, 1, dilation, dilation, 1) || B < 1 || H < 1 || W < 1) return 0;
+  if (!x || !wpack || !out || (mean == nullptr) != (var == nullptr) || geometry < 0 || geometry > 3) return 0;
+  if ((reinterpret_cast<uintptr_t>(x) | reinterpret_cast<uintptr_t>(wpack)) & 15) return 0;
+  if ((int64_t)H * W > 2147483647 || dilation > (1 << 24)) return 0;
+  const int64_t M = (int64_t)B * H * W;
+  hipStream_t st = as_stream(stream);
+  const uint4 *bp = static_cast<const uint4 *>(wpack);
+  switch (activation) {
+    case SKD_ACT_NONE: return launch3g<SKD_ACT_NONE>(x, bp, out, conv_bias, mean, var, weight, bias, eps, slope, M, H, W, Cin, Cout, dilation, geometry, st);
+    case SKD_ACT_RELU: return launch3g<SKD_ACT_RELU>(x, bp, out, conv_bias, mean, var, weight, bias, eps, slope, M, H, W, Cin, Cout, dilation, geometry, st);
+    case SKD_ACT_LEAKY_RELU: return launch3g<SKD_ACT_LEAKY_RELU>(x, bp, out, conv_bias, mean, var, weight, bias, eps, slope, M, H, W, Cin, Cout, dilation, geometry, st);
+    default: return 0;
+  }
+}
+
+}
diff --git a/structure_knowledge_distillation_amd/csrc/conv_split_dev.hpp b/structure_knowledge_distillation_amd/csrc/conv_split_dev.hpp
--- /dev/null
+++ b/structure_knowledge_distillation_amd/csrc/conv_split_dev.hpp
@@ -0,0 +1,125 @@
+#pragma once
+#include <atomic>
+
+#include "skd_common.hpp"
+
+namespace skd {
+
+typedef float f32x16 __attribute__((ext_vector_type(16)));
+typedef __bf16 bf16x8 __attribute__((ext_vector_type(8)));
+typedef __bf16 bf16x2 __attribute__((ext_vector_type(2)));
+typedef float f32x2 __attribute__((ext_vector_type(2)));
+
+constexpr int kTM = 128, kTN = 128, kBK = 16, kMinWG = 3;
+constexpr int kQK = kBK / 4;
+constexpr int kRPP = kThreads / kQK;
+constexpr int kRB = kTN / kRPP;
+constexpr int kPlaneChunks = 2 * 128;
+constexpr int kOperandChunks = 3 * kPlaneChunks;
+constexpr int kStageChunks = 2 * kOperandChunks;
+constexpr size_t kConvLds = sizeof(uint4) * 2 * kStageChunks;
+
+__device__ __forceinline__ float inv_std_of(float var, float eps) { return (var != 0.f || eps != 0.f) ? 1.f / sqrtf(var + eps) : 0.f; }
+
+__device__ __forceinline__ uint32_t pack_bf16(float x, float y) {
+  const f32x2 v = {x, y};
+  return __builtin_bit_cast(uint32_t, __builtin_convertvector(v, bf16x2));
+}
+__device__ __forceinline__ float bf16_lo(uint32_t u) { return __uint_as_float(u << 16); }
+__device__ __forceinline__ float bf16_hi(uint32_t u) { return __uint_as_float(u & 0xffff0000u); }
+
+__device__ __forceinline__ void split4(float4 v, uint2 &p0, uint2 &p1, uint2 &p2) {
+  p0.x = pack_bf16(v.x, v.y);
+  p0.y = pack_bf16(v.z, v.w);
+  v.x -= bf16_lo(p0.x); v.y -= bf16_hi(p0.x); v.z -= bf16_lo(p0.y); v.w -= bf16_hi(p0.y);
+  p1.x = pack_bf16(v.x, v.y);
+  p1.y = pack_bf16(v.z, v.w);
+  v.x -= bf16_lo(p1.x); v.y -= bf16_hi(p1.x); v.z -= bf16_lo(p1.y); v.w -= bf16_hi(p1.y);
+  p2.x = pack_bf16(v.x, v.y);
+  p2.y = pack_bf16(v.z, v.w);
+}
+__device__ __forceinline__ void split_store(float4 v, uint2 *dst) {
+  uint2 p0, p1, p2;
+  split4(v, p0, p1, p2);
+  dst[0] = p0;
+  dst[2 * kPlaneChunks] = p1;
+  dst[4 * kPlaneChunks] = p2;
+}
+
+__device__ __forceinline__ int plane_slot(int row, int gkq) {
+  const int kh = gkq >> 3;
+  return 2 * (kh * 128 + (row ^ (kh * 4))) + ((gkq >> 2) & 1);
+}
+
+template <int TM>
+__device__ __forceinline__ void tile_mma(const uint4 *stage, f32x16 (&lo)[TM / 64][2], f32x16 (&hi)[TM / 64][2]) {
+  constexpr int WM = TM / 64;
+  const int lane = threadIdx.x & (kWave - 1), wid = threadIdx.x / kWave;
+  const int wi = (wid >> 1) * (TM / 2), wj = (wid & 1) * 64;
+  const int half = lane >> 5, r = lane & 31;
+  const uint4 *pa = stage + half * 128 + ((wi + r) ^ (half * 4));
+  const uint4 *pb = stage + kOperandChunks + half * 128 + ((wj + r) ^ (half * 4));
+  bf16x8 a[WM][3], b[2][3];
+#pragma unroll
+  for (int p = 0; p < 3; ++p) {
+#pragma unroll
+    for (int i = 0; i < WM; ++i) a[i][p] = __builtin_bit_cast(bf16x8, pa[p * kPlaneChunks + 32 * i]);
+#pragma unroll
+    for (int j = 0; j < 2; ++j) b[j][p] = __builtin_bit_cast(bf16x8, pb[p * kPlaneChunks + 32 * j]);
+  }
+  constexpr int kPA[6] = {0, 1, 2, 0, 1, 0}, kPB[6] = {2, 1, 0, 1, 0, 0};
+#pragma unroll
+  for (int t = 0; t < 6; ++t)
+#pragma unroll
+    for (int i = 0; i < WM; ++i)
+#pragma unroll
+      for (int j = 0; j < 2; ++j) {
+        f32x16 &dst = t < 5 ? lo[i][j] : hi[i][j];
+        dst = __builtin_amdgcn_mfma_f32_32x32x16_bf16(a[i][kPA[t]], b[j][kPB[t]], dst, 0, 0, 0);
+      }
+}
+template <int TM>
+__device__ __forceinline__ void tile_mma(const uint4 *stage, f32x16 (&acc)[TM / 64][2]) { tile_mma<TM>(stage, acc, acc); }
+
+template <int ACT, bool HAS_RES, bool FULL, bool NT>
+__device__ __forceinline__ void store_block(const f32x16 &acc, const float *__restrict__ R, float *__restrict__ Y, int64_t row0,
+                                            int col, int64_t M, int N, float mu, float is, float ga, float be, float slope) {
+  const int lane = threadIdx.x & (kWave - 1);
+  float rv[16];
+  int64_t off[16];
+#pragma unroll
+  for (int q = 0; q < 16; ++q) {
+    const int64_t row = row0 + (q & 3) + 8 * (q >> 2) + 4 * (lane >> 5);
+    off[q] = row * N + col;
+    rv[q] = 0.f;
+    if (HAS_RES && (FULL || row < M)) rv[q] = NT ? __builtin_nontemporal_load(R + off[q]) : R[off[q]];
+  }
+#pragma unroll
+  for (int q = 0; q < 16; ++q) {
+    const int64_t row = row0 + (q & 3) + 8 * (q >> 2) + 4 * (lane >> 5);
+    float z = ((acc[q] - mu) * is) * ga + be;
+    if (HAS_RES) z += rv[q];
+    if (ACT == SKD_ACT_RELU) z = z < 0.f ? 0.f : z;
+    if (ACT == SKD_ACT_LEAKY_RELU) z = z < 0.f ? z * slope : z;
+    if (FULL || row < M) {
+      if (NT) __builtin_nontemporal_store(z, Y + off[q]);
+      else Y[off[q]] = z;
+    }
+  }
+}
+
+inline int cu_count(hipStream_t st) {
+  static std::atomic<int> cus[64];
+  int dev = -1;
+  if (hipStreamGetDevice(st, &dev) != hipSuccess) {
+    (void)hipGetLastError();
+    if (hipGetDevice(&dev) != hipSuccess) return 0;
+  }
+  if (dev < 0 || dev >= 64) return 0;
+  int n = cus[dev].load(std::memory_order_relaxed);
+  if (n == 0 && hipDeviceGetAttribute(&n, hipDeviceAttributeMultiprocessorCount, dev) == hipSuccess && n > 0)
+    cus[dev].store(n, std::memory_order_relaxed);
+  return n > 0 ? n : 0;
+}
+
+}
diff --git a/structure_knowledge_distillation_amd/functional.py b/structure_knowledge_distillation_amd/functional.py
--- a/structure_knowledge_distillation_amd/functional.py
+++ b/structure_knowledge_distillation_amd/functional.py
@@ -1,4 +1,5 @@
 import ctypes
+import types
 
 import torch
 from torch.autograd import Function
@@ -283,7 +284,7 @@
         and _is_cl(feats) and 3 * sum(sizes) <= 64 and len(sizes) <= 4
 
 
-def ppm_fold_bottleneck(priors, feats, weight, cache=None):
+def ppm_fold_bottleneck(priors, feats, weight, cache=None, split3x3=False):
     import torch.nn.functional as F
     cm = priors[0].shape[1]
     n_prior = len(priors) * cm
@@ -298,7 +299,11 @@
         if cache is not None and not (torch.is_grad_enabled() and weight.requires_grad):
             cache["key"], cache["mats"] = key, mats
     wf, w_all = mats
-    base = F.conv2d(feats, wf, None, 1, 1)
+    if split3x3 and cache is not None and _conv3x3_split_ok(feats, weight[:, n_prior:], 1, 1, 1, 1):
+        owner = cache.setdefault("pack3x3", types.SimpleNamespace())
+        base = conv3x3_split_eval(feats, conv3x3_pack_weights(None, weight[:, n_prior:], owner), cout)
+    else:
+        base = F.conv2d(feats, wf, None, 1, 1)
     p_all = torch.cat([_cl(p).permute(0, 2, 3, 1).reshape(-1, cm) for p in priors], 0)
     return _PPMFold.apply(base, sizes, torch.mm(p_all, w_all))
 
@@ -485,6 +490,73 @@
     _lib.check(_lib.get().skd_conv1x1_abn_nhwc(b * h * w, k, n, x.data_ptr(), wt.data_ptr(), _lib.ptr(residual), out.data_ptr(),
                                                running_mean.data_ptr(), running_var.data_ptr(), _lib.ptr(weight), _lib.ptr(bias),
                                                float(eps), act, float(slope), _lib.stream_of(x)), "skd_conv1x1_abn_nhwc")
+    return out
+
+
+def _pair(v):
+    return tuple(v) if isinstance(v, (tuple, list)) else (v, v)
+
+
+def _conv3x3_split_ok(x, weight, stride, padding, dilation, groups):
+    if torch.is_grad_enabled() or not _lib.has_entry("skd_conv3x3_split_nhwc"):
+        return False
+    if not (x.is_cuda and x.dtype == torch.float32 and x.dim() == 4 and x.is_contiguous(memory_format=torch.channels_last)
+            and x.data_ptr() % 16 == 0):
+        return False
+    if not (weight.dim() == 4 and tuple(weight.shape[2:]) == (3, 3) and weight.dtype == torch.float32
+            and weight.device == x.device and x.shape[1] == weight.shape[1] * groups):
+        return False
+    return bool(_lib.get().skd_conv3x3_split_supported(int(weight.shape[1]), int(weight.shape[0]), stride, padding, dilation, groups))
+
+
+def conv3x3_split_supported(x, conv):
+    if not (isinstance(conv, torch.nn.Conv2d) and conv.padding_mode == "zeros" and not isinstance(conv.padding, str)):
+        return False
+    s, p, d = _pair(conv.stride), _pair(conv.padding), _pair(conv.dilation)
+    if s[0] != s[1] or p[0] != p[1] or d[0] != d[1]:
+        return False
+    return _conv3x3_split_ok(x, conv.weight, s[0], p[0], d[0], conv.groups)
+
+
+def conv3x3_pack_weights(conv, weight=None, owner=None):
+    w = conv.weight if weight is None else weight
+    owner = conv if owner is None else owner
+    if torch.is_grad_enabled() and w.requires_grad:
+        raise RuntimeError("conv3x3_pack_weights is for frozen (no-grad) convolutions")
+    key = (w.data_ptr(), w._version, tuple(w.shape), tuple(w.stride()))
+    cached = getattr(owner, "_skd_conv3x3_pack", None)
+    if cached is not None and cached[0] == key:
+        return cached[1]
+    _lib.require_device(w)
+    cout, cin = int(w.shape[0]), int(w.shape[1])
+    lib = _lib.get()
+    nbytes = int(lib.skd_conv3x3_split_pack_bytes(cin, cout))
+    if nbytes <= 0 or tuple(w.shape[2:]) != (3, 3) or w.dtype != torch.float32:
+        raise ValueError("conv3x3_pack_weights: unsupported weight %s" % (tuple(w.shape),))
+    pack = torch.empty((nbytes,), dtype=torch.uint8, device=w.device)
+    sn, sc, sy, sx = (int(v) for v in w.stride())
+    _lib.check(lib.skd_conv3x3_split_pack_weights(cin, cout, w.data_ptr(), sn, sc, sy, sx, pack.data_ptr(), nbytes,
+                                                  _lib.stream_of(pack)), "skd_conv3x3_split_pack_weights")
+    owner._skd_conv3x3_pack = (key, pack, w.untyped_storage())
+    return pack
+
+
+def conv3x3_split_eval(x, pack, cout, dilation=1, conv_bias=None, bn=None, activation="none", geometry=0):
+    if torch.is_grad_enabled() and x.requires_grad:
+        raise RuntimeError("conv3x3_split_eval is inference-only")
+    _lib.require_device(x, pack, conv_bias)
+    act = {"none": 0, "leaky_relu": 1, "relu": 3}[activation]
+    b, cin, h, w = x.shape
+    if pack.numel() != _lib.get().skd_conv3x3_split_pack_bytes(cin, cout):
+        raise ValueError("conv3x3_split_eval: the pack is not that of a (%d, %d, 3, 3) weight" % (cout, cin))
+    out = _new_cl(x, b, cout, h, w)
+    mean = var = gamma = beta = None
+    eps, slope = 0.0, 0.01
+    if bn is not None:
+        mean, var, gamma, beta, eps, slope = bn.running_mean, bn.running_var, bn.weight, bn.bias, float(bn.eps), float(bn.slope)
+    _lib.check(_lib.get().skd_conv3x3_split_nhwc(b, h, w, cin, cout, int(dilation), x.data_ptr(), pack.data_ptr(), out.data_ptr(),
+                                                 _lib.ptr(conv_bias), _lib.ptr(mean), _lib.ptr(var), _lib.ptr(gamma), _lib.ptr(beta),
+                                                 eps, act, slope, int(geometry), _lib.stream_of(x)), "skd_conv3x3_split_nhwc")
     return out
 
 
diff --git a/structure_knowledge_distillation_amd/networks/pspnet_combine.py b/structure_knowledge_distillation_amd/networks/pspnet_combine.py
--- a/structure_knowledge_distillation_amd/networks/pspnet_combine.py
+++ b/structure_knowledge_distillation_amd/networks/pspnet_combine.py
@@ -20,6 +20,9 @@
 HEAD_KERNEL = True
 STEM_FUSED = True
 PSP_FOLD = True
+CONV3X3_SPLIT = True
+CONV3X3_SPLIT_MIN_CIN = 256
+SPLIT_REDUCE = True
 
 
 def _fused_tail(x):
@@ -28,6 +31,19 @@
 
 def _blas_tail(module, x):
     return BLAS_TAILS and not module.training and not torch.is_grad_enabled()
+
+
+def _conv1x1_bn_eval(x, conv, bn, relu):
+    if (SPLIT_REDUCE and not (conv.in_channels == 512 and conv.out_channels == 128)
+            and getattr(bn, "activation", None) == "none" and SF.conv1x1_abn_supported(x, conv)):
+        return SF.conv1x1_abn_eval(x, conv.weight, bn.running_mean, bn.running_var, bn.weight, bn.bias, bn.eps,
+                                   "relu" if relu else "none")
+    return SF.conv1x1_bn_blas(x, conv, bn, relu=relu)
+
+
+def _conv3x3_split(x, conv):
+    return (CONV3X3_SPLIT and conv.in_channels >= CONV3X3_SPLIT_MIN_CIN and not conv.training
+            and SF.conv3x3_split_supported(x, conv))
 
 
 class _ClassifierConvFn(torch.autograd.Function):
@@ -114,10 +130,13 @@
         if _fused(self, x):
             blas = _blas_tail(self, x)
             if blas and SF.blas_1x1_bn_supported(x, self.conv1):
-                out = SF.conv1x1_bn_blas(x, self.conv1, self.bn1, relu=True)
+                out = _conv1x1_bn_eval(x, self.conv1, self.bn1, relu=True)
             else:
                 out = self.bn1.forward_relu(self.conv1(x))
-            c2 = self.conv2(out)
+            if _conv3x3_split(out, self.conv2):
+                c2 = SF.conv3x3_split_eval(out, SF.conv3x3_pack_weights(self.conv2), self.conv2.out_channels, self.conv2.dilation[0])
+            else:
+                c2 = self.conv2(out)
             tail = (not self.training and _fused_tail(x) and SF.conv1x1_abn_supported(c2, self.conv3) and self.conv3.in_channels <= 512
                     and getattr(self.bn2, "activation", None) == "none" and getattr(self.bn3, "activation", None) == "none")
             if not tail:
@@ -126,7 +145,7 @@
                 residual = x
             elif (blas and len(self.downsample) == 2 and SF.blas_1x1_bn_supported(x, self.downsample[0])
                   and getattr(self.downsample[1], "activation", None) == "none"):
-                residual = SF.conv1x1_bn_blas(x, self.downsample[0], self.downsample[1], relu=False)
+                residual = _conv1x1_bn_eval(x, self.downsample[0], self.downsample[1], relu=False)
             else:
                 residual = self.downsample(x)
             if tail:
@@ -186,7 +205,8 @@
                     and all(p.shape[1] == priors[0].shape[1] for p in priors)):
                 if not hasattr(self, "_fold_cache"):
                     self._fold_cache = {}
-                out = SF.ppm_fold_bottleneck(priors, feats, conv.weight, self._fold_cache)
+                out = SF.ppm_fold_bottleneck(priors, feats, conv.weight, self._fold_cache,
+                                             split3x3=CONV3X3_SPLIT and not self.training and feats.shape[1] >= CONV3X3_SPLIT_MIN_CIN)
                 return self.bottleneck[2](self.bottleneck[1](out))
             return self.bottleneck(SF.ppm_concat(priors, feats))
         h, w = feats.size(2), feats.size(3)
@@ -242,6 +262,15 @@
             mods.append(block(self.inplanes, planes, dilation=dilation, multi_grid=grid(i)))
         return nn.Sequential(*mods)
 
+    def _dsn_head(self, x3):
+        conv, bn = self.dsn[0], self.dsn[1]
+        if (not self.training and not torch.is_grad_enabled() and getattr(bn, "activation", None) in ("none", "relu", "leaky_relu")
+                and hasattr(bn, "running_mean") and _conv3x3_split(x3, conv)):
+            y = SF.conv3x3_split_eval(x3, SF.conv3x3_pack_weights(conv), conv.out_channels, conv.dilation[0], conv.bias, bn,
+                                      bn.activation)
+            return self.dsn[3](y)
+        return self.dsn(x3)
+
     def forward(self, x):
         if _fused(self, x) and not self.training and getattr(self.bn3, "activation", None) == "none":
             x = self.bn1.forward_relu(self.conv1(x))
@@ -268,10 +297,10 @@
             x_feat_after_psp = self.pspmodule(x4)
             x = self.head(x_feat_after_psp)
             self.dsn_last(x, x_feat_after_psp)
-            x_dsn = self.dsn(x3)
+            x_dsn = self._dsn_head(x3)
             return [x, x_dsn, x_feat_after_psp, x4, x3, x2, x1]
         else:
-            x_dsn = self.dsn(x3)
+            x_dsn = self._dsn_head(x3)
         x4 = self.layer4(x3)
         x_feat_after_psp = self.pspmodule(x4)
         x = self.head(x_feat_after_psp)
```

Measured after the change: 142.4 images/sec (median of 6 runs). +7.1%, better.
